# yuanzhi-zhu/DiffPIR

Hardware: AMD Instinct MI355X
Metric: restored images/sec @100 NFE, 256x256 (higher is better)
Workload: dtype f32 (GEMMs as 3 x f16 MFMA on hi/lo-split fp32 operands, fp32 accumulate; exact-fp32-MFMA mode in alt_precision); 1 GPU; configs[1]: ffhq topology 256x256 deblur (61x61 Gaussian PSF), 100 NFE, batch 16/GPU, device Philox noise, hipGraph=on; global_batch=16, nfe=100, collective=none

## Files before the change

### diffpir_amd/_lib.py

```python
from __future__ import annotations

import ctypes as C
import os

_HERE = os.path.dirname(os.path.abspath(__file__))
LIB_PATH = os.environ.get("DIFFPIR_LIB") or os.path.join(_HERE, "csrc", "libdiffpir_hip.so")
ABI_VERSION = 2



class UNetDesc(C.Structure):
    _fields_ = [("image_size", C.c_int32), ("in_channels", C.c_int32), ("model_channels", C.c_int32),
                ("out_channels", C.c_int32), ("num_res_blocks", C.c_int32), ("num_head_channels", C.c_int32),
                ("n_channel_mult", C.c_int32), ("channel_mult", C.c_float * 8),
                ("n_attention_ds", C.c_int32), ("attention_ds", C.c_int32 * 8), ("num_classes", C.c_int32)]


class Tensor(C.Structure):
    _fields_ = [("name", C.c_char_p), ("data", C.c_void_p), ("ndim", C.c_int32), ("shape", C.c_int64 * 4)]


class Step(C.Structure):
    _fields_ = [("t", C.c_int32), ("last", C.c_int32), ("c1", C.c_float), ("c2", C.c_float), ("tau", C.c_float),
                ("sa_t", C.c_float), ("s1m_t", C.c_float), ("sa_p", C.c_float),
                ("k1", C.c_float), ("q", C.c_float), ("es", C.c_float), ("k2", C.c_float)]


class LoopDesc(C.Structure):
    _fields_ = [("task", C.c_int32), ("B", C.c_int32), ("H", C.c_int32), ("W", C.c_int32), ("sf", C.c_int32),
                ("kh", C.c_int32), ("kw", C.c_int32), ("in_iter", C.c_int32), ("gamma", C.c_float),
                ("guidance", C.c_float), ("sa_start", C.c_float), ("s1m_start", C.c_float),
                ("y_dev", C.c_void_p), ("k_dev", C.c_void_p), ("mask_dev", C.c_void_p), ("labels_host", C.c_void_p),
                ("noise_init_dev", C.c_void_p), ("noise_n1_dev", C.c_void_p), ("noise_n2_dev", C.c_void_p),
                ("seed", C.c_uint64), ("image_offset", C.c_int64), ("use_graph", C.c_int32),
                ("skip_dead_final_eval", C.c_int32), ("generate_mode", C.c_int32), ("first_order", C.c_int32),
                ("noise_rp_dev", C.c_void_p), ("ddim_sample", C.c_int32)]


class InpaintRow(C.Structure):
    _fields_ = [("t", C.c_int32), ("last", C.c_int32), ("pos", C.c_int32), ("back", C.c_int32),
                ("c1", C.c_float), ("c2", C.c_float), ("tau", C.c_float), ("sa_t", C.c_float), ("s1m_t", C.c_float), ("sa_p", C.c_float),
                ("k1", C.c_float), ("q", C.c_float), ("es", C.c_float), ("k2", C.c_float),
                ("sae", C.c_float), ("sb", C.c_float), ("sa_n", C.c_float), ("s1m_n", C.c_float),
                ("mix_next", C.c_int32), ("reserved", C.c_int32)]


class DpsCoef(C.Structure):
    _fields_ = [("pc1", C.c_float), ("pc2", C.c_float), ("min_log", C.c_float), ("max_log", C.c_float), ("sa_prev", C.c_float), ("s1m_prev", C.c_float)]


class PSampleCoef(C.Structure):
    _fields_ = [("c1", C.c_float), ("c2", C.c_float), ("pc1", C.c_float), ("pc2", C.c_float), ("min_log", C.c_float), ("max_log", C.c_float),
                ("ddim", C.c_int32), ("sa_prev", C.c_float), ("s1m_prev", C.c_float)]


class DegradeDesc(C.Structure):
    _fields_ = [("task", C.c_int32), ("B", C.c_int32), ("H", C.c_int32), ("W", C.c_int32), ("sf", C.c_int32),
                ("kh", C.c_int32), ("kw", C.c_int32), ("noise_level_img", C.c_float), ("seed", C.c_uint64), ("image_offset", C.c_int64)]


class Conv3Desc(C.Structure):
    _fields_ = ([(n, C.c_int32) for n in ("B", "ca", "cb", "Cout", "H", "W", "mode", "res_mode", "scaled", "prologue", "route", "split",
                                          "defer", "Cout2")] +
                [(n, C.c_void_p) for n in ("xa", "xb", "w", "bias", "res", "prm", "gamma", "beta", "film", "gamma2", "beta2", "w2", "bias2",
                                           "out", "stat_out", "out2")] +
                [(n, C.c_int32) for n in ("stat_kind_out", "path_out", "ksplit_out", "reserved")])


class Conv9Desc(C.Structure):
    _fields_ = ([(n, C.c_int32) for n in ("B", "Cin", "Cout", "H", "W", "res_mode", "hop", "Cout2")] +
                [(n, C.c_void_p) for n in ("x", "w", "bias", "res", "prm", "gamma2", "beta2", "film2", "w2", "bias2", "out", "stat_out", "out2")] +
                [(n, C.c_int32) for n in ("ran_out", "iters")] + [("ms_out", C.c_double)])


PROF_CLASSES = 8
PROF_NAMES = ["conv3x3", "conv1x1", "groupnorm_stats", "attention", "fft_prox", "elementwise", "unet_forward", "loop_graph"]

SIGNATURES = {
    "dpir_version": (C.c_int, []),
    "dpir_device_count": (C.c_int, [C.POINTER(C.c_int)]),
    "dpir_create": (C.c_int, [C.c_int, C.POINTER(C.c_void_p)]),
    "dpir_destroy": (None, [C.c_void_p]),
    "dpir_last_error": (C.c_char_p, [C.c_void_p]),
    "dpir_sync": (C.c_int, [C.c_void_p]),
    "dpir_stream": (C.c_void_p, [C.c_void_p]),
    "dpir_malloc": (C.c_int, [C.c_void_p, C.c_size_t, C.POINTER(C.c_void_p)]),
    "dpir_free": (C.c_int, [C.c_void_p, C.c_void_p]),
    "dpir_h2d": (C.c_int, [C.c_void_p, C.c_void_p, C.c_void_p, C.c_size_t]),
    "dpir_d2h": (C.c_int, [C.c_void_p, C.c_void_p, C.c_void_p, C.c_size_t]),
    "dpir_d2d": (C.c_int, [C.c_void_p, C.c_void_p, C.c_void_p, C.c_size_t]),
    "dpir_load_unet": (C.c_int, [C.c_void_p, C.POINTER(UNetDesc), C.POINTER(Tensor), C.c_int]),
    "dpir_set_precision": (C.c_int, [C.c_void_p, C.c_int]),
    "dpir_unet_forward": (C.c_int, [C.c_void_p, C.c_void_p, C.c_void_p, C.c_void_p, C.c_void_p, C.c_int, C.c_int, C.c_int]),
    "dpir_model_fn_xstart": (C.c_int, [C.c_void_p, C.c_void_p, C.c_int, C.c_float, C.c_float, C.c_void_p, C.c_void_p,
                                       C.c_int, C.c_int, C.c_int]),
    "dpir_enable_grad": (C.c_int, [C.c_void_p, C.c_int]),
    "dpir_unet_vjp": (C.c_int, [C.c_void_p, C.c_void_p, C.c_void_p, C.c_void_p, C.c_void_p, C.c_void_p, C.c_void_p, C.c_int, C.c_int, C.c_int]),
    "dpir_run_dps_loop": (C.c_int, [C.c_void_p, C.POINTER(LoopDesc), C.POINTER(Step), C.POINTER(DpsCoef), C.c_int, C.c_int, C.c_float,
                                    C.c_void_p, C.c_void_p, C.c_float, C.c_void_p, C.c_void_p]),
    "dpir_p_sample": (C.c_int, [C.c_void_p, C.c_void_p, C.c_int, C.POINTER(PSampleCoef), C.c_void_p, C.c_void_p, C.c_void_p, C.c_void_p, C.c_int, C.c_int, C.c_int]),
    "dpir_eps_from_xstart": (C.c_int, [C.c_void_p, C.c_void_p, C.c_void_p, C.c_float, C.c_float, C.c_int, C.c_void_p, C.c_size_t]),
    "dpir_grad_and_value": (C.c_int, [C.c_void_p, C.c_int, C.c_void_p, C.c_void_p, C.c_int, C.c_void_p, C.c_void_p, C.c_int, C.c_int, C.c_int]),
    "dpir_blur_reflect": (C.c_int, [C.c_void_p, C.c_void_p, C.c_void_p, C.c_int, C.c_int, C.c_float, C.c_float, C.c_void_p, C.c_int, C.c_int, C.c_int]),
    "dpir_blur_reflect_adjoint": (C.c_int, [C.c_void_p, C.c_void_p, C.c_void_p, C.c_int, C.c_int, C.c_float, C.c_void_p, C.c_int, C.c_int, C.c_int]),
    "dpir_grad_and_value_blur": (C.c_int, [C.c_void_p, C.c_int, C.c_void_p, C.c_void_p, C.c_void_p, C.c_int, C.c_int, C.c_void_p, C.c_void_p,
                                           C.c_int, C.c_int, C.c_int]),
    "dpir_run_deblur_grad_loop": (C.c_int, [C.c_void_p, C.POINTER(LoopDesc), C.POINTER(Step), C.POINTER(DpsCoef), C.c_int, C.c_int, C.c_float,
                                            C.c_void_p, C.c_void_p, C.c_void_p, C.c_void_p]),
    "dpir_unet_read_tap": (C.c_int, [C.c_void_p, C.c_char_p, C.c_void_p, C.c_size_t, C.POINTER(C.c_size_t)]),
    "dpir_prox_fft_precalc": (C.c_int, [C.c_void_p, C.c_void_p, C.c_void_p, C.c_int, C.c_int, C.c_int, C.c_int, C.c_int,
                                        C.c_int, C.POINTER(C.c_void_p)]),
    "dpir_prox_free": (None, [C.c_void_p, C.c_void_p]),
    "dpir_prox_read": (C.c_int, [C.c_void_p, C.c_void_p, C.c_int, C.c_void_p, C.c_size_t]),
    "dpir_data_solution": (C.c_int, [C.c_void_p, C.c_void_p, C.c_void_p, C.c_float, C.c_void_p]),
    "dpir_prox_fft_apply": (C.c_int, [C.c_void_p, C.c_void_p, C.c_void_p, C.c_float, C.c_float]),
    "dpir_set_prox_launch": (C.c_int, [C.c_void_p, C.c_int]),
    "dpir_prox_fft_apply_timed": (C.c_int, [C.c_void_p, C.c_void_p, C.c_void_p, C.c_float, C.c_float, C.c_int, C.c_int, C.POINTER(C.c_float)]),
    "dpir_prox_mask": (C.c_int, [C.c_void_p, C.c_void_p, C.c_void_p, C.c_void_p, C.c_float, C.c_float, C.c_int, C.c_int, C.c_int]),
    "dpir_resize_down": (C.c_int, [C.c_void_p, C.c_void_p, C.c_void_p, C.c_int, C.c_int, C.c_int, C.c_int]),
    "dpir_prox_ibp": (C.c_int, [C.c_void_p, C.c_void_p, C.c_void_p, C.c_float, C.c_float, C.c_int, C.c_int, C.c_int, C.c_int, C.c_int]),
    "dpir_bicubic_up": (C.c_int, [C.c_void_p, C.c_void_p, C.c_void_p, C.c_int, C.c_int, C.c_int, C.c_int]),
    "dpir_renoise": (C.c_int, [C.c_void_p, C.c_void_p, C.c_void_p, C.POINTER(Step), C.c_void_p, C.c_void_p, C.c_int, C.c_int, C.c_int]),
    "dpir_repaint_mix": (C.c_int, [C.c_void_p, C.c_void_p, C.c_void_p, C.c_void_p, C.c_void_p, C.c_void_p, C.c_int, C.c_int, C.c_int]),
    "dpir_finalize": (C.c_int, [C.c_void_p, C.c_void_p, C.c_void_p, C.c_void_p, C.c_int, C.c_int, C.c_int]),
    "dpir_randn": (C.c_int, [C.c_void_p, C.c_void_p, C.c_uint64, C.c_uint64, C.c_int64, C.c_int, C.c_int, C.c_int, C.c_int]),
    "dpir_ewise": (C.c_int, [C.c_void_p, C.c_int, C.c_void_p, C.c_void_p, C.c_size_t, C.c_float, C.c_void_p, C.c_size_t]),
    "dpir_comm_unique_id": (C.c_int, [C.c_void_p]),
    "dpir_comm_version": (C.c_int, [C.POINTER(C.c_int)]),
    "dpir_device_info": (C.c_int, [C.c_void_p, C.c_char_p, C.c_size_t]),
    "dpir_comm_init": (C.c_int, [C.c_void_p, C.c_int, C.c_int, C.c_void_p]),
    "dpir_allgather_results": (C.c_int, [C.c_void_p, C.c_void_p, C.c_void_p, C.c_size_t]),
    "dpir_comm_allreduce_max": (C.c_int, [C.c_void_p, C.POINTER(C.c_double)]),
    "dpir_comm_barrier": (C.c_int, [C.c_void_p]),
    "dpir_comm_destroy": (C.c_int, [C.c_void_p]),
    "dpir_degrade": (C.c_int, [C.c_void_p, C.POINTER(DegradeDesc), C.c_void_p, C.c_void_p, C.c_void_p, C.c_void_p, C.c_void_p]),
    "dpir_metrics": (C.c_int, [C.c_void_p, C.c_void_p, C.c_void_p, C.c_int, C.c_int, C.c_int, C.c_void_p, C.c_void_p]),
    "dpir_run_loop": (C.c_int, [C.c_void_p, C.POINTER(LoopDesc), C.POINTER(Step), C.c_int, C.c_void_p, C.c_void_p]),
    "dpir_inpaint_step": (C.c_int, [C.c_void_p, C.c_void_p, C.c_void_p, C.c_int, C.c_void_p, C.c_void_p, C.POINTER(InpaintRow), C.c_int, C.c_float,
                                    C.c_void_p, C.c_void_p, C.c_void_p, C.c_void_p, C.c_uint64, C.c_int64, C.c_int, C.c_void_p, C.c_int, C.c_int, C.c_int]),
    "dpir_run_inpaint_loop": (C.c_int, [C.c_void_p, C.POINTER(LoopDesc), C.POINTER(InpaintRow), C.c_int, C.c_void_p, C.c_void_p, C.c_void_p]),
    "dpir_prof_enable": (C.c_int, [C.c_void_p, C.c_int]),
    "dpir_prof_reset": (C.c_int, [C.c_void_p]),
    "dpir_prof_read": (C.c_int, [C.c_void_p, C.POINTER(C.c_double), C.POINTER(C.c_int64)]),
    "dpir_graph_cache_size": (C.c_int, [C.c_void_p]),
    "dpir_unet_flops": (C.c_double, [C.c_void_p, C.c_int, C.c_int]),
    "dpir_unet_flops_class": (C.c_double, [C.c_void_p, C.c_int, C.c_int, C.c_int]),
}

_lib = None


class EngineLibraryError(RuntimeError):
    pass


DEBUG_LIB_PATH = os.path.join(_HERE, "csrc", "libdiffpir_dbg.so")
_dbg = None


def load_debug():
    global _dbg
    if _dbg is not None:
        return _dbg
    load()
    if not os.path.exists(DEBUG_LIB_PATH):
        raise EngineLibraryError(f"{DEBUG_LIB_PATH} not found: `make -C diffpir_amd/csrc` builds it next to the product library")
    d = C.CDLL(DEBUG_LIB_PATH)
    d.dpir_debug_conv_bench.argtypes = [C.c_void_p] + [C.c_int] * 10 + [C.POINTER(C.c_double)]
    d.dpir_debug_conv7_emit_supported.argtypes = [C.c_void_p] + [C.c_int] * 4 + [C.POINTER(C.c_int)]
    d.dpir_debug_victim.argtypes = [C.c_void_p, C.c_int, C.c_int, C.c_int, C.c_longlong, C.c_int, C.POINTER(C.c_ulonglong)]
    d.dpir_debug_victim_alu.argtypes = [C.c_void_p, C.c_int, C.c_int, C.c_int, C.c_int, C.POINTER(C.c_ulonglong)]
    for fn in (d.dpir_debug_victim_fft_pk, d.dpir_debug_victim_fft_nopk):
        fn.argtypes = [C.c_void_p, C.c_int, C.c_int, C.c_int, C.POINTER(C.c_ulonglong)]
    d.dpir_debug_conv7_check.argtypes = [C.c_void_p] + [C.c_int] * 10 + [C.POINTER(C.c_double), C.POINTER(C.c_double), C.POINTER(C.c_ulonglong),
                                                                        C.POINTER(C.c_float), C.POINTER(C.c_int)]
    d.dpir_debug_conv5_layer.argtypes = [C.c_void_p] + [C.c_int] * 7 + [C.c_void_p] * 7 + [C.POINTER(C.c_int)]
    d.dpir_debug_conv5_layer.restype = C.c_int
    d.dpir_debug_conv3_layer.argtypes = [C.c_void_p, C.POINTER(Conv3Desc)]
    d.dpir_debug_conv3_layer.restype = C.c_int
    d.dpir_debug_conv9_layer.argtypes = [C.c_void_p, C.POINTER(Conv9Desc)]
    d.dpir_debug_conv9_layer.restype = C.c_int
    for n in ("dpir_debug_conv_bench", "dpir_debug_victim", "dpir_debug_victim_alu", "dpir_debug_victim_fft_pk", "dpir_debug_victim_fft_nopk",
              "dpir_debug_conv7_check"):
        getattr(d, n).restype = C.c_int
    _dbg = d
    return d


def load():
    global _lib
    if _lib is not None:
        return _lib
    if not os.path.exists(LIB_PATH):
        raise EngineLibraryError(
            f"{LIB_PATH} not found: build it with `python -c 'import __graft_entry__ as g; g.build()'` "
            f"or `make -C diffpir_amd/csrc`.  There is no CPU fallback.")
    try:
        import torch
    except ImportError:
        pass
    try:
        lib = C.CDLL(LIB_PATH)
    except OSError as ex:
        raise EngineLibraryError(f"cannot load {LIB_PATH}: {ex}") from ex
    for name, (res, args) in SIGNATURES.items():
        try:
            fn = getattr(lib, name)
        except AttributeError as ex:
            raise EngineLibraryError(f"{LIB_PATH} does not export {name}") from ex
        fn.restype = res
        fn.argtypes = args
    if lib.dpir_version() != ABI_VERSION:
        raise EngineLibraryError("ABI version mismatch")
    _lib = lib
    return lib
```

### diffpir_amd/csrc/dbg_conv.hip

```cpp
#include "engine.h"
#include "conv6_params.h"
#include "conv9.h"
#include "../../include/diffpir_debug.h"
#include <string.h>
#include <vector>
using namespace dpir;
static int fail(dpir_engine* e, const Status& s) {
    if (e) e->last_error = s.msg;
    return s.code;
}
#define API_TRY(e, expr)                          \
    do {                                          \
        Status _s = (expr);                       \
        if (!_s.ok()) return fail((e), _s);       \
    } while (0)
#define API_HIP(e, expr)                                                                  \
    do {                                                                                  \
        hipError_t _h = (expr);                                                           \
        if (_h != hipSuccess)                                                             \
            return fail((e), Status{DPIR_ERR_HIP, std::string(#expr) + ": " + hipGetErrorString(_h)}); \
    } while (0)

__global__ void dbg_bitdiff_kernel(const float* a, const float* b, size_t n, unsigned long long* out) {
    unsigned long long cnt = 0; unsigned mx = 0;
    for (size_t i = (size_t)blockIdx.x * blockDim.x + threadIdx.x; i < n; i += (size_t)gridDim.x * blockDim.x) {
        const float x = a[i], y = b[i];
        if (__builtin_bit_cast(unsigned, x) != __builtin_bit_cast(unsigned, y)) {
            ++cnt;
            const float d = fabsf(x - y);
            const unsigned u = d == d ? __builtin_bit_cast(unsigned, d) : 0x7fc00000u;
            mx = u > mx ? u : mx;
        }
    }
    if (cnt) { atomicAdd(&out[0], cnt); atomicMax(&out[1], (unsigned long long)mx); }
}

extern "C" {
int dpir_debug_conv_bench(dpir_engine* e, int B, int Cin, int Cout, int H, int W, int ks, int mode, int with_prm,
                          int dbg, int iters, double* ms_out) {
    if (!e || !ms_out || iters <= 0) return DPIR_ERR_INVALID;
    (void)hipSetDevice(e->device);
    int taps = ks * ks, coutp = round_up(Cout, 64), cinp = round_up(Cin, 16);
    float *x = nullptr, *w = nullptr, *bias = nullptr, *out = nullptr, *partial = nullptr; float4* prm = nullptr;
    API_TRY(e, e->ws.getT("dbg#x", (size_t)B * Cin * H * W, &x));
    API_TRY(e, e->ws.getT("dbg#w", (size_t)cinp * taps * coutp, &w));
    API_TRY(e, e->ws.getT("dbg#b", (size_t)coutp, &bias));
    API_TRY(e, e->ws.getT("dbg#o", (size_t)B * Cout * H * W, &out));
    API_TRY(e, e->ws.getT("dbg#prm", (size_t)B * Cin, &prm));
    API_TRY(e, e->ws.getT("conv#partial", (size_t)16 * 1024 * 1024, &partial));
    API_TRY(e, launch_randn(e->stream, x, 1, 1, 0, 1, (size_t)B * Cin * H * W));
    API_TRY(e, launch_randn(e->stream, w, 2, 1, 0, 1, (size_t)cinp * taps * coutp));
    API_TRY(e, launch_randn(e->stream, bias, 3, 1, 0, 1, (size_t)coutp));
    API_TRY(e, launch_randn(e->stream, reinterpret_cast<float*>(prm), 4, 1, 0, 1, (size_t)B * Cin * 4));
    ConvArgs a;
    a.src.a = x; a.src.ca = Cin; a.src.Hs = H; a.src.Ws = W; a.src.mode = 0; a.src.prm = with_prm ? prm : nullptr;
    a.w = w; a.bias = bias; a.out = out; a.B = B; a.Cin = Cin; a.Cout = Cout; a.CoutP = coutp; a.H = H; a.W = W; a.ks = ks;
    a.partial = partial; a.partial_capacity = (size_t)16 * 1024 * 1024;
    const void* w16 = nullptr; float w16_scale = 1.f;
    if (dbg != 0) {
        std::vector<float> hw((size_t)Cout * Cin * taps);
        for (size_t i = 0; i < hw.size(); ++i) hw[i] = (float)((i * 2654435761u) % 2001) / 1000.0f * 0.05f - 0.05f;
        std::vector<uint16_t> w16v;
        w16_scale = ks == 1 ? pack_weights_f16x3_1x1(hw.data(), Cout, Cin, w16v) : pack_weights_conv6(hw.data(), Cout, Cin, w16v);
        void* wp = nullptr;
        API_TRY(e, e->ws.get("dbg#w16", w16v.size() * 2, &wp));
        API_HIP(e, hipMemcpy(wp, w16v.data(), w16v.size() * 2, hipMemcpyHostToDevice));
        w16 = wp;
    }
    Conv5Args a5;
    Conv6Args a6;
    const bool use5 = dbg != 0 && ks == 1, use6 = dbg != 0 && ks == 3;
    if (use5) {
        a5.src = CatSrc{x, Cin, nullptr, 0}; a5.prm = a.src.prm; a5.w16 = w16; a5.w16_scale = w16_scale; a5.bias = bias; a5.out = out;
        a5.B = B; a5.Cout = Cout; a5.H = H; a5.W = W; a5.x1 = e->precision == 2;
    }
    if (use6) {
        int C8 = 2 * ((Cin + 15) / 16);
        size_t plane = (size_t)B * C8 * H * W * 16;
        char* s16 = nullptr;
        API_TRY(e, e->ws.getT("dbg#s16", 2 * plane, &s16));
        API_TRY(e, launch_act_split(e->stream, CatSrc{x, Cin, nullptr, 0}, a.src.prm, 0, B, H, W, s16, s16 + plane));
        a6.xhi = s16; a6.xlo = s16 + plane; a6.w16 = w16; a6.w16_scale = w16_scale; a6.bias = bias; a6.out = out;
        a6.B = B; a6.Cin = Cin; a6.Cout = Cout; a6.H = H; a6.W = W; a6.partial = partial; a6.partial_capacity = a.partial_capacity;
        a6.x1 = e->precision == 2;
    }
    auto run_once = [&]() -> Status {
        if (use5) return launch_conv5(e->stream, a5);
        if (use6) {
            if (dbg == 1) DPIR_TRY(launch_act_split(e->stream, CatSrc{x, Cin, nullptr, 0}, a.src.prm, 0, B, H, W, const_cast<void*>(a6.xhi), const_cast<void*>(a6.xlo)));
            return launch_conv6(e->stream, a6);
        }
        return launch_conv(e->stream, a);
    };
    API_TRY(e, run_once());
    hipEvent_t e0, e1;
    API_HIP(e, hipEventCreate(&e0)); API_HIP(e, hipEventCreate(&e1));
    API_HIP(e, hipEventRecord(e0, e->stream));
    for (int i = 0; i < iters; ++i) API_TRY(e, run_once());
    API_HIP(e, hipEventRecord(e1, e->stream));
    API_HIP(e, hipEventSynchronize(e1));
    float ms = 0; API_HIP(e, hipEventElapsedTime(&ms, e0, e1));
    (void)hipEventDestroy(e0); (void)hipEventDestroy(e1);
    *ms_out = ms / iters;
    return DPIR_OK;
}

int dpir_debug_conv7_check(dpir_engine* e, int B, int Cin, int Cout, int H, int W, int res_mode, int x1, int split, int scaled, int iters,
                            double* ms6_out, double* ms7_out, unsigned long long* mismatches_out, float* maxdiff_out, int* ksplit_out) {
    if (!e || !ms6_out || !ms7_out || !mismatches_out || !maxdiff_out || !ksplit_out || iters <= 0 || res_mode < -1 || res_mode > 2) return DPIR_ERR_INVALID;
    (void)hipSetDevice(e->device);
    if (!conv6_supported(H, W) || W < 32) return fail(e, invalid("conv7 check: conv6 only has the 8 x 32 geometry (W >= 32) to compare with"));
    const size_t nx = (size_t)B * Cin * H * W, no = (size_t)B * Cout * H * W;
    const size_t nres = res_mode == 1 ? no / 4 : (res_mode == 2 ? no * 4 : no);
    const int slots = conv6_stat_slots(H, W);
    const size_t nst = (size_t)B * Cout * slots;
    const size_t pcap = (size_t)16 * no;
    float *x = nullptr, *bias = nullptr, *o6 = nullptr, *o7 = nullptr, *res = nullptr, *p6 = nullptr, *p7 = nullptr, *scale = nullptr;
    float2 *st6 = nullptr, *st7 = nullptr;
    unsigned long long* cmp = nullptr;
    API_TRY(e, e->ws.getT("c7#x", nx, &x));
    API_TRY(e, e->ws.getT("c7#b", (size_t)round_up(Cout, 64), &bias));
    API_TRY(e, e->ws.getT("c7#o6", no, &o6));
    API_TRY(e, e->ws.getT("c7#o7", no, &o7));
    API_TRY(e, e->ws.getT("c7#res", nres, &res));
    API_TRY(e, e->ws.getT("c7#st6", nst, &st6));
    API_TRY(e, e->ws.getT("c7#st7", nst, &st7));
    API_TRY(e, e->ws.getT("c7#cmp", (size_t)2, &cmp));
    API_TRY(e, e->ws.getT("c7#scale", (size_t)4, &scale));
    if (split) { API_TRY(e, e->ws.getT("c7#p6", pcap, &p6)); API_TRY(e, e->ws.getT("c7#p7", pcap, &p7)); }
    API_TRY(e, launch_randn(e->stream, x, 11, 1, 0, 1, nx));
    API_TRY(e, launch_randn(e->stream, bias, 12, 1, 0, 1, (size_t)round_up(Cout, 64)));
    API_TRY(e, launch_randn(e->stream, res, 13, 1, 0, 1, nres));
    const float quarter = 0.25f;
    API_HIP(e, hipMemcpyAsync(scale, &quarter, 4, hipMemcpyHostToDevice, e->stream));
    std::vector<float> hw((size_t)Cout * Cin * 9);
    for (size_t i = 0; i < hw.size(); ++i) hw[i] = (float)((i * 2654435761u) % 2001) / 1000.0f * 0.05f - 0.05f;
    std::vector<uint16_t> w16v;
    const float w16_scale = pack_weights_conv6(hw.data(), Cout, Cin, w16v);
    void* wp = nullptr;
    API_TRY(e, e->ws.get("c7#w16", w16v.size() * 2, &wp));
    API_HIP(e, hipMemcpy(wp, w16v.data(), w16v.size() * 2, hipMemcpyHostToDevice));
    const int chunks = (Cin + 15) / 16, C8 = 2 * chunks;
    const size_t plane = (size_t)B * C8 * H * W * 16;
    char* s16 = nullptr;
    API_TRY(e, e->ws.getT("c7#s16", 2 * plane, &s16));
    API_TRY(e, launch_act_split(e->stream, CatSrc{x, Cin, nullptr, 0}, nullptr, 0, B, H, W, s16, x1 ? nullptr : s16 + plane));
    Conv6Args a6;
    a6.xhi = s16; a6.xlo = x1 ? nullptr : s16 + plane; a6.w16 = wp; a6.w16_scale = w16_scale; a6.bias = bias;
    a6.B = B; a6.Cin = Cin; a6.Cout = Cout; a6.H = H; a6.W = W; a6.x1 = x1 != 0;
    if (res_mode >= 0) { a6.res = res; a6.res_mode = res_mode; }
    if (scaled) a6.out_scale_dev = scale;
    a6.out = o6; a6.stat = st6; a6.force_kernel = 6;
    if (split) { a6.partial = p6; a6.partial_capacity = pcap; }
    Conv6K k;
    k.xhi = reinterpret_cast<const char*>(a6.xhi); k.xlo = reinterpret_cast<const char*>(a6.xlo);
    k.w16 = reinterpret_cast<const char*>(wp); k.bias = bias; k.out = o7; k.res = a6.res; k.res_mode = a6.res_mode;
    k.B = B; k.Cout = Cout; k.H = H; k.W = W; k.n_chunks_total = chunks; k.C8 = C8;
    k.out_scale = 1.0f / w16_scale; k.out_scale_dev = a6.out_scale_dev; k.zeros = nullptr;
    const int geo = W >= 32 ? 0 : (W >= 16 ? 1 : 2);
    const int tw = geo == 0 ? 32 : (geo == 1 ? 16 : 8), th = geo == 0 ? 8 : (geo == 1 ? 16 : 8), ti = geo == 2 ? 4 : 1;
    k.tiles_x = (W + tw - 1) / tw; k.tiles_y = (H + th - 1) / th;
    const int n_ptiles = k.tiles_x * k.tiles_y * ((B + ti - 1) / ti);
    k.n_co_blocks = (Cout + 127) / 128;
    const int blocks = n_ptiles * k.n_co_blocks;
    int S = 1;
    if (split && blocks < 384) {
        S = (512 + blocks - 1) / blocks;
        if (S > chunks / 2) S = chunks / 2;
        if (S > 16) S = 16;
        if (S < 1) S = 1;
        if ((size_t)S * no > pcap) S = 1;
    }
    k.chunks_per_split = (chunks + S - 1) / S;
    S = (chunks + k.chunks_per_split - 1) / k.chunks_per_split;
    k.ksplit = S; k.partial = S > 1 ? p7 : nullptr;
    k.stat = S == 1 ? st7 : nullptr; k.stat_slots = S == 1 ? slots : 0;
    *ksplit_out = S;
    API_HIP(e, hipMemsetAsync(o6, 0xFF, no * 4, e->stream));
    API_HIP(e, hipMemsetAsync(o7, 0x7F, no * 4, e->stream));
    API_HIP(e, hipMemsetAsync(st6, 0xFF, nst * 8, e->stream));
    API_HIP(e, hipMemsetAsync(st7, 0x7F, nst * 8, e->stream));
    if (split) { API_HIP(e, hipMemsetAsync(p6, 0xFF, (size_t)S * no * 4, e->stream)); API_HIP(e, hipMemsetAsync(p7, 0x7F, (size_t)S * no * 4, e->stream)); }
    API_HIP(e, hipMemsetAsync(cmp, 0, 16, e->stream));
    int k6 = 0;
    PendingConv pend;
    API_TRY(e, launch_conv6(e->stream, a6, &k6, &pend));
    if ((S > 1) != (k6 == 3) || (S > 1 && pend.ksplit != S)) return fail(e, Status{DPIR_ERR_INVALID, "conv7 check: the split rule of launch_conv6 changed"});
    API_TRY(e, launch_conv7(e->stream, k, blocks * S, x1 != 0));
    API_HIP(e, hipGetLastError());
    if (S > 1) {
        hipLaunchKernelGGL(dbg_bitdiff_kernel, dim3(2048), dim3(256), 0, e->stream, p6, p7, (size_t)S * no, cmp);
    } else {
        hipLaunchKernelGGL(dbg_bitdiff_kernel, dim3(2048), dim3(256), 0, e->stream, o6, o7, no, cmp);
        hipLaunchKernelGGL(dbg_bitdiff_kernel, dim3(256), dim3(256), 0, e->stream, reinterpret_cast<const float*>(st6), reinterpret_cast<const float*>(st7), nst * 2, cmp);
    }
    unsigned long long h[2] = {0, 0};
    API_HIP(e, hipMemcpyAsync(h, cmp, 16, hipMemcpyDeviceToHost, e->stream));
    API_HIP(e, hipStreamSynchronize(e->stream));
    *mismatches_out = h[0];
    const unsigned mb = (unsigned)h[1];
    *maxdiff_out = __builtin_bit_cast(float, mb);
    hipEvent_t e0, e1, e2;
    API_HIP(e, hipEventCreate(&e0)); API_HIP(e, hipEventCreate(&e1)); API_HIP(e, hipEventCreate(&e2));
    for (int i = 0; i < 3; ++i) { API_TRY(e, launch_conv6(e->stream, a6, &k6, &pend)); API_TRY(e, launch_conv7(e->stream, k, blocks * S, x1 != 0)); }
    API_HIP(e, hipEventRecord(e0, e->stream));
    for (int i = 0; i < iters; ++i) API_TRY(e, launch_conv6(e->stream, a6, &k6, &pend));
    API_HIP(e, hipEventRecord(e1, e->stream));
    for (int i = 0; i < iters; ++i) API_TRY(e, launch_conv7(e->stream, k, blocks * S, x1 != 0));
    API_HIP(e, hipEventRecord(e2, e->stream));
    API_HIP(e, hipEventSynchronize(e2));
    float m6 = 0, m7 = 0;
    API_HIP(e, hipEventElapsedTime(&m6, e0, e1)); API_HIP(e, hipEventElapsedTime(&m7, e1, e2));
    (void)hipEventDestroy(e0); (void)hipEventDestroy(e1); (void)hipEventDestroy(e2);
    *ms6_out = m6 / iters; *ms7_out = m7 / iters;
    return DPIR_OK;
}

int dpir_debug_conv5_layer(dpir_engine* e, int B, int ca, int cb, int Cout, int H, int W, int tile, const float* xa, const float* xb,
                           const float* w, const float* bias, const float* prm, const float* res, float* out, int* path_out) {
    if (!e || !xa || !w || !bias || !out || !path_out || B <= 0 || ca <= 0 || cb < 0 || (cb > 0 && !xb) || Cout <= 0 || tile < 0 || tile > 2) return DPIR_ERR_INVALID;
    if (e->precision == 0) return fail(e, invalid("conv5 layer: the engine is in f32 mode"));
    (void)hipSetDevice(e->device);
    const int C = ca + cb, HW = H * W;
    const size_t na = (size_t)B * ca * HW, nb = (size_t)B * cb * HW, no = (size_t)B * Cout * HW;
    float *dxa = nullptr, *dxb = nullptr, *dbias = nullptr, *dout = nullptr, *dres = nullptr, *dw = nullptr, *partial = nullptr; float4* dprm = nullptr;
    API_TRY(e, e->ws.getT("c5#xa", na, &dxa));
    API_TRY(e, e->ws.getT("c5#xb", nb + 1, &dxb));
    API_TRY(e, e->ws.getT("c5#b", (size_t)round_up(Cout, 64), &dbias));
    API_TRY(e, e->ws.getT("c5#o", no, &dout));
    API_TRY(e, e->ws.getT("c5#res", no, &dres));
    API_TRY(e, e->ws.getT("c5#prm", (size_t)B * C, &dprm));
    API_HIP(e, hipMemcpy(dxa, xa, na * 4, hipMemcpyHostToDevice));
    if (cb) API_HIP(e, hipMemcpy(dxb, xb, nb * 4, hipMemcpyHostToDevice));
    API_HIP(e, hipMemset(dbias, 0, (size_t)round_up(Cout, 64) * 4));
    API_HIP(e, hipMemcpy(dbias, bias, (size_t)Cout * 4, hipMemcpyHostToDevice));
    if (prm) API_HIP(e, hipMemcpy(dprm, prm, (size_t)B * C * 16, hipMemcpyHostToDevice));
    if (res) API_HIP(e, hipMemcpy(dres, res, no * 4, hipMemcpyHostToDevice));
    API_HIP(e, hipMemset(dout, 0xFF, no * 4));
    std::vector<uint16_t> w16v;
    const float w16_scale = pack_weights_f16x3_1x1(w, Cout, C, w16v);
    void* wp = nullptr;
    API_TRY(e, e->ws.get("c5#w16", w16v.size() * 2, &wp));
    API_HIP(e, hipMemcpy(wp, w16v.data(), w16v.size() * 2, hipMemcpyHostToDevice));
    const bool has_prm = prm != nullptr;
    const bool use5 = !(has_prm && C % 16) && (tile != 0 || conv5_supported(B, Cout, H, W, has_prm) || conv5_small_supported(B, ca, cb, Cout, H, W, has_prm));
    Status st;
    if (use5) {
        Conv5Args a5;
        a5.src = CatSrc{dxa, ca, cb ? dxb : nullptr, cb}; a5.prm = has_prm ? dprm : nullptr; a5.w16 = wp; a5.w16_scale = w16_scale;
        a5.bias = dbias; a5.out = dout; a5.res = res ? dres : nullptr; a5.B = B; a5.Cout = Cout; a5.H = H; a5.W = W;
        a5.x1 = e->precision == 2; a5.force_tile = tile;
        *path_out = tile ? tile : (conv5_small_supported(B, ca, cb, Cout, H, W, has_prm) ? 2 : 1);
        st = launch_conv5(e->stream, a5);
    } else {
        const int coutp = round_up(Cout, 64), cinp = round_up(C, 16);
        std::vector<float> packed((size_t)cinp * coutp, 0.f);
        for (int co = 0; co < Cout; ++co)
            for (int ci = 0; ci < C; ++ci) packed[(size_t)ci * coutp + co] = w[(size_t)co * C + ci];
        API_TRY(e, e->ws.getT("c5#w", packed.size(), &dw));
        API_HIP(e, hipMemcpy(dw, packed.data(), packed.size() * 4, hipMemcpyHostToDevice));
        API_TRY(e, e->ws.getT("conv#partial", (size_t)16 * 1024 * 1024, &partial));
        ConvArgs a;
        a.src.a = dxa; a.src.ca = ca; a.src.b = cb ? dxb : nullptr; a.src.cb = cb; a.src.Hs = H; a.src.Ws = W; a.src.mode = 0;
        a.src.prm = has_prm ? dprm : nullptr;
        a.w = dw; a.bias = dbias; a.out = dout; a.res = res ? dres : nullptr; a.res_mode = 0;
        a.B = B; a.Cin = C; a.Cout = Cout; a.CoutP = coutp; a.H = H; a.W = W; a.ks = 1;
        a.partial = partial; a.partial_capacity = (size_t)16 * 1024 * 1024;
        *path_out = 0;
        st = launch_conv(e->stream, a);
    }
    API_TRY(e, st);
    API_HIP(e, hipStreamSynchronize(e->stream));
    API_HIP(e, hipMemcpy(out, dout, no * 4, hipMemcpyDeviceToHost));
    return DPIR_OK;
}

int dpir_debug_conv3_layer(dpir_engine* e, dpir_debug_conv3_desc* d) {
    if (!e || !d) return DPIR_ERR_INVALID;
    d->path_out = -1; d->ksplit_out = 0; d->stat_kind_out = 0;
    const int B = d->B, ca = d->ca, cb = d->cb, Cout = d->Cout, H = d->H, W = d->W, mode = d->mode, C = ca + cb;
    if (!d->xa || !d->w || !d->bias || !d->out || B <= 0 || ca <= 0 || cb < 0 || (cb > 0 && !d->xb) || Cout <= 0 || H <= 0 || W <= 0 || mode < 0 || mode > 2 ||
        d->res_mode < -1 || d->res_mode > 2 || (d->res_mode >= 0 && !d->res) || d->prologue < 0 || d->prologue > 2 ||
        (d->route != 0 && d->route != 6 && d->route != 7 && d->route != 8))
        return fail(e, invalid("conv3 layer: bad descriptor"));
    if (d->prologue == 1 && !d->prm) return fail(e, invalid("conv3 layer: prologue 1 needs the table"));
    if (d->prologue == 2 && (!d->gamma || !d->beta)) return fail(e, invalid("conv3 layer: prologue 2 needs gamma and beta"));
    if (mode == 1 && ((H | W) & 1)) return fail(e, invalid("conv3 layer: a nearest-up source needs an even output size"));
    if (d->res_mode == 1 && ((H | W) & 1)) return fail(e, invalid("conv3 layer: a half-resolution residual needs an even output size"));
    if (d->defer && (!d->split || (d->route != 0 && d->route != 7) || !d->gamma2 || !d->beta2 || !d->w2 || !d->bias2 || !d->out2 || d->Cout2 <= 0))
        return fail(e, invalid("conv3 layer: defer needs split, route 0 or 7 and the second stage's operands"));
    (void)hipSetDevice(e->device);
    const int Hs = mode == 1 ? H / 2 : (mode == 2 ? H * 2 : H), Ws = mode == 1 ? W / 2 : (mode == 2 ? W * 2 : W);
    const size_t HWs = (size_t)Hs * Ws, HW = (size_t)H * W;
    const size_t na = (size_t)B * ca * HWs, nb = (size_t)B * cb * HWs, no = (size_t)B * Cout * HW;
    const size_t nres = d->res_mode == 1 ? no / 4 : (d->res_mode == 2 ? no * 4 : no);
    const int coutp = round_up(Cout, 64);
    float *dxa = nullptr, *dxb = nullptr, *dbias = nullptr, *dout = nullptr, *dres = nullptr, *scale = nullptr; float4* dprm = nullptr;
    API_TRY(e, e->ws.getT("c3#xa", na, &dxa));
    API_TRY(e, e->ws.getT("c3#xb", nb + 1, &dxb));
    API_TRY(e, e->ws.getT("c3#b", (size_t)coutp, &dbias));
    API_TRY(e, e->ws.getT("c3#o", no, &dout));
    API_TRY(e, e->ws.getT("c3#res", nres, &dres));
    API_TRY(e, e->ws.getT("c3#prm", (size_t)B * C, &dprm));
    API_TRY(e, e->ws.getT("c3#scale", (size_t)4, &scale));
    API_HIP(e, hipMemcpy(dxa, d->xa, na * 4, hipMemcpyHostToDevice));
    if (cb) API_HIP(e, hipMemcpy(dxb, d->xb, nb * 4, hipMemcpyHostToDevice));
    API_HIP(e, hipMemset(dbias, 0, (size_t)coutp * 4));
    API_HIP(e, hipMemcpy(dbias, d->bias, (size_t)Cout * 4, hipMemcpyHostToDevice));
    if (d->prologue == 1) API_HIP(e, hipMemcpy(dprm, d->prm, (size_t)B * C * 16, hipMemcpyHostToDevice));
    if (d->res_mode >= 0) API_HIP(e, hipMemcpy(dres, d->res, nres * 4, hipMemcpyHostToDevice));
    const float quarter = 0.25f;
    API_HIP(e, hipMemcpy(scale, &quarter, 4, hipMemcpyHostToDevice));
    API_HIP(e, hipMemset(dout, 0xFF, no * 4));
    const float* res = d->res_mode >= 0 ? dres : nullptr;
    const int res_mode = d->res_mode >= 0 ? d->res_mode : 0;
    const CatSrc src{dxa, ca, cb ? dxb : nullptr, cb};
    const bool x1 = e->precision == 2;
    const bool f16path = e->precision != 0 && conv6_supported(H, W);
    const size_t pcap = (size_t)16 * no;
    float* partial = nullptr;
    if (d->split) {
        API_TRY(e, e->ws.getT("c3#partial", pcap, &partial));
        API_HIP(e, hipMemset(partial, 0xFF, pcap * 4));
    }

    if (d->route == 8) {
        if (e->precision == 0) return fail(e, invalid("conv3 layer: conv8 needs an f16 engine"));
        if (d->prologue != 1 || cb || mode != 0 || res || d->scaled || d->split) return fail(e, invalid("conv3 layer: conv8 takes a table prologue, one source, no resampling, no residual"));
        if (!conv8_supported(B, C, Cout, H, W)) return fail(e, invalid("conv8: shape not supported"));
        std::vector<uint16_t> w8;
        const float w8_scale = pack_weights_conv8(d->w, Cout, C, w8);
        void* wp = nullptr;
        API_TRY(e, e->ws.get("c3#w8", w8.size() * 2, &wp));
        API_HIP(e, hipMemcpy(wp, w8.data(), w8.size() * 2, hipMemcpyHostToDevice));
        Conv8Args a8;
        a8.x = dxa; a8.prm = dprm; a8.w = wp; a8.w_scale = w8_scale; a8.bias = dbias; a8.out = dout;
        a8.B = B; a8.C = C; a8.Cout = Cout; a8.H = H; a8.W = W; a8.range_ctr = e->range_ctr; a8.x1 = x1;
        a8.silu = d->prm[3] != 0.f;
        API_TRY(e, launch_conv8(e->stream, a8));
        API_HIP(e, hipStreamSynchronize(e->stream));
        API_HIP(e, hipMemcpy(d->out, dout, no * 4, hipMemcpyDeviceToHost));
        d->path_out = 8;
        return DPIR_OK;
    }

    if (!f16path) {
        if (d->route != 0) return fail(e, invalid("conv3 layer: conv6 / conv7 cannot be forced here (f32 engine or a shape the f16 path refuses)"));
        if (d->prologue == 2) return fail(e, Status{DPIR_ERR_UNSUPPORTED, "conv3 layer: gn_act_small only feeds the f16 path"});
        if (d->scaled || d->defer) return fail(e, invalid("conv3 layer: the fp32 kernel has no device output scale and no deferred combine"));
        const int cinp = round_up(C, 16);
        std::vector<float> packed((size_t)cinp * 9 * coutp, 0.f);
        for (int co = 0; co < Cout; ++co)
            for (int ci = 0; ci < C; ++ci)
                for (int t = 0; t < 9; ++t) packed[((size_t)ci * 9 + t) * coutp + co] = d->w[((size_t)co * C + ci) * 9 + t];
        float* dw = nullptr;
        API_TRY(e, e->ws.getT("c3#w", packed.size(), &dw));
        API_HIP(e, hipMemcpy(dw, packed.data(), packed.size() * 4, hipMemcpyHostToDevice));
        ConvArgs a;
        a.src.a = dxa; a.src.ca = ca; a.src.b = cb ? dxb : nullptr; a.src.cb = cb; a.src.Hs = Hs; a.src.Ws = Ws; a.src.mode = mode;
        a.src.prm = d->prologue == 1 ? dprm : nullptr;
        a.w = dw; a.bias = dbias; a.out = dout; a.res = res; a.res_mode = res_mode;
        a.B = B; a.Cin = C; a.Cout = Cout; a.CoutP = coutp; a.H = H; a.W = W; a.ks = 3;
        a.partial = partial; a.partial_capacity = partial ? pcap : 0;
        API_TRY(e, launch_conv(e->stream, a));
        API_HIP(e, hipStreamSynchronize(e->stream));
        API_HIP(e, hipMemcpy(d->out, dout, no * 4, hipMemcpyDeviceToHost));
        d->path_out = 0;
        return DPIR_OK;
    }

    const int C8 = 2 * ((C + 15) / 16);
    const size_t plane = (size_t)B * C8 * HW * 16;
    char* s16 = nullptr;
    API_TRY(e, e->ws.getT("c3#s16", 2 * plane, &s16));
    API_HIP(e, hipMemset(s16, 0xFF, 2 * plane));
    if (d->prologue == 2) {
        if (C % 16 || !gn_act_small_supported(C, Hs, Ws, mode)) return fail(e, Status{DPIR_ERR_UNSUPPORTED, "conv3 layer: gn_act_small refuses this shape"});
        float *dg = nullptr, *db = nullptr, *df = nullptr;
        API_TRY(e, e->ws.getT("c3#gamma", (size_t)C, &dg));
        API_TRY(e, e->ws.getT("c3#beta", (size_t)C, &db));
        API_TRY(e, e->ws.getT("c3#film", (size_t)B * 2 * C, &df));
        API_HIP(e, hipMemcpy(dg, d->gamma, (size_t)C * 4, hipMemcpyHostToDevice));
        API_HIP(e, hipMemcpy(db, d->beta, (size_t)C * 4, hipMemcpyHostToDevice));
        if (d->film) API_HIP(e, hipMemcpy(df, d->film, (size_t)B * 2 * C * 4, hipMemcpyHostToDevice));
        GnActArgs ga;
        ga.src = src; ga.gamma = dg; ga.beta = db;
        ga.film = d->film ? df : nullptr; ga.film_stride = 2 * C; ga.film_off = 0; ga.fstep = nullptr; ga.frows = 2 * C;
        ga.silu = true; ga.mode = mode; ga.B = B; ga.Hs = Hs; ga.Ws = Ws;
        ga.hi = s16; ga.lo = x1 ? nullptr : s16 + plane; ga.range_ctr = e->range_ctr;
        API_TRY(e, launch_gn_act_small(e->stream, ga));
    } else {
        API_TRY(e, launch_act_split(e->stream, src, d->prologue == 1 ? dprm : nullptr, mode, B, H, W, s16, x1 ? nullptr : s16 + plane, e->range_ctr));
    }
    std::vector<uint16_t> w16v;
    const float w16_scale = pack_weights_conv6(d->w, Cout, C, w16v);
    void* wp = nullptr;
    API_TRY(e, e->ws.get("c3#w16", w16v.size() * 2, &wp));
    API_HIP(e, hipMemcpy(wp, w16v.data(), w16v.size() * 2, hipMemcpyHostToDevice));
    Conv6Args a6;
    a6.x1 = x1;
    a6.xhi = s16; a6.xlo = s16 + plane; a6.w16 = wp; a6.w16_scale = w16_scale;
    a6.bias = dbias; a6.out = dout; a6.res = res; a6.res_mode = res_mode;
    a6.B = B; a6.Cin = C; a6.Cout = Cout; a6.H = H; a6.W = W;
    a6.partial = partial; a6.partial_capacity = partial ? pcap : 0;
    a6.force_kernel = d->route;
    if (d->scaled) a6.out_scale_dev = scale;
    const int slots = conv6_stat_slots(H, W);
    float2* st = nullptr; double2* sp = nullptr;
    const size_t nst = (size_t)B * Cout * slots;
    if (slots > 0 && Cout % 32 == 0) {
        API_TRY(e, e->ws.getT("c3#st", nst, &st));
        API_TRY(e, e->ws.getT("c3#sp", (size_t)B * Cout, &sp));
        API_HIP(e, hipMemset(st, 0xFF, nst * 8));
        API_HIP(e, hipMemset(sp, 0xFF, (size_t)B * Cout * 16));
    }
    a6.stat = st; a6.stat_plane = sp;
    int kind = 0, kernel = 0;
    PendingConv pc;
    API_TRY(e, launch_conv6(e->stream, a6, &kind, d->defer ? &pc : nullptr, &kernel));
    d->path_out = kernel; d->stat_kind_out = kind;
    d->ksplit_out = kind == 3 ? pc.ksplit : 1;
    if (d->split && !d->defer) {
        PendingConv probe;
        Conv6Args b6 = a6;
        float* o2 = nullptr;
        API_TRY(e, e->ws.getT("c3#o_again", no, &o2));
        b6.out = o2;
        int k2 = 0;
        API_HIP(e, hipStreamSynchronize(e->stream));
        std::vector<float> first(no);
        API_HIP(e, hipMemcpy(first.data(), dout, no * 4, hipMemcpyDeviceToHost));
        API_TRY(e, launch_conv6(e->stream, b6, &k2, &probe));
        d->ksplit_out = k2 == 3 ? probe.ksplit : 1;
        if (k2 == 3) API_TRY(e, launch_conv6_resolve(e->stream, probe));
        API_HIP(e, hipStreamSynchronize(e->stream));
        std::vector<float> again(no);
        API_HIP(e, hipMemcpy(again.data(), o2, no * 4, hipMemcpyDeviceToHost));
        if (memcmp(first.data(), again.data(), no * 4) != 0) return fail(e, Status{DPIR_ERR_STATE, "conv3 layer: two identical split-K launches disagree"});
    }
    if (d->defer) {
        if (kind != 3) return fail(e, invalid("conv3 layer: defer was asked for but launch_conv6 did not split this launch"));
        const int Cn = Cout, Co2 = d->Cout2;
        if (Cn % 16 || !gn_act_small_supported(Cn, H, W, 0)) return fail(e, Status{DPIR_ERR_UNSUPPORTED, "conv3 layer: gn_act_small refuses the second stage"});
        const int C8b = 2 * ((Cn + 15) / 16);
        const size_t plane2 = (size_t)B * C8b * HW * 16, no2 = (size_t)B * Co2 * HW;
        char* s16b = nullptr; float *dg = nullptr, *db = nullptr, *dbias2 = nullptr, *dout2 = nullptr;
        API_TRY(e, e->ws.getT("c3#s16b", 2 * plane2, &s16b));
        API_TRY(e, e->ws.getT("c3#gamma2", (size_t)Cn, &dg));
        API_TRY(e, e->ws.getT("c3#beta2", (size_t)Cn, &db));
        API_TRY(e, e->ws.getT("c3#b2", (size_t)round_up(Co2, 64), &dbias2));
        API_TRY(e, e->ws.getT("c3#o2", no2, &dout2));
        API_HIP(e, hipMemset(s16b, 0xFF, 2 * plane2));
        API_HIP(e, hipMemcpy(dg, d->gamma2, (size_t)Cn * 4, hipMemcpyHostToDevice));
        API_HIP(e, hipMemcpy(db, d->beta2, (size_t)Cn * 4, hipMemcpyHostToDevice));
        API_HIP(e, hipMemset(dbias2, 0, (size_t)round_up(Co2, 64) * 4));
        API_HIP(e, hipMemcpy(dbias2, d->bias2, (size_t)Co2 * 4, hipMemcpyHostToDevice));
        API_HIP(e, hipMemset(dout2, 0xFF, no2 * 4));
        GnActArgs ga;
        ga.src = CatSrc{dout, Cn, nullptr, 0}; ga.pend = pc; ga.gamma = dg; ga.beta = db;
        ga.silu = true; ga.mode = 0; ga.B = B; ga.Hs = H; ga.Ws = W;
        ga.hi = s16b; ga.lo = x1 ? nullptr : s16b + plane2; ga.range_ctr = e->range_ctr;
        API_TRY(e, launch_gn_act_small(e->stream, ga));
        std::vector<uint16_t> w16b;
        const float w16b_scale = pack_weights_conv6(d->w2, Co2, Cn, w16b);
        void* wp2 = nullptr;
        API_TRY(e, e->ws.get("c3#w16b", w16b.size() * 2, &wp2));
        API_HIP(e, hipMemcpy(wp2, w16b.data(), w16b.size() * 2, hipMemcpyHostToDevice));
        Conv6Args c6;
        c6.x1 = x1; c6.xhi = s16b; c6.xlo = s16b + plane2; c6.w16 = wp2; c6.w16_scale = w16b_scale;
        c6.bias = dbias2; c6.out = dout2; c6.B = B; c6.Cin = Cn; c6.Cout = Co2; c6.H = H; c6.W = W;
        API_TRY(e, launch_conv6(e->stream, c6));
        API_HIP(e, hipStreamSynchronize(e->stream));
        API_HIP(e, hipMemcpy(d->out2, dout2, no2 * 4, hipMemcpyDeviceToHost));
    }
    API_HIP(e, hipStreamSynchronize(e->stream));
    API_HIP(e, hipMemcpy(d->out, dout, no * 4, hipMemcpyDeviceToHost));
    if (d->stat_out && (kind == 1 || kind == 2)) {
        if (kind == 1) {
            std::vector<float2> hs(nst);
            API_HIP(e, hipMemcpy(hs.data(), st, nst * 8, hipMemcpyDeviceToHost));
            for (size_t pl = 0; pl < (size_t)B * Cout; ++pl) {
                double s1 = 0.0, s2 = 0.0;
                for (int k = 0; k < slots; ++k) { s1 += (double)hs[pl * slots + k].x; s2 += (double)hs[pl * slots + k].y; }
                d->stat_out[2 * pl] = s1; d->stat_out[2 * pl + 1] = s2;
            }
        } else {
            API_HIP(e, hipMemcpy(d->stat_out, sp, (size_t)B * Cout * 16, hipMemcpyDeviceToHost));
        }
    }
    return DPIR_OK;
}

int dpir_debug_conv9_layer(dpir_engine* e, dpir_debug_conv9_desc* d) {
    if (!e || !d) return DPIR_ERR_INVALID;
    d->ran_out = 0;
    const int B = d->B, Cin = d->Cin, Cout = d->Cout, H = d->H, W = d->W;
    if (!d->x || !d->w || !d->bias || B <= 0 || Cin <= 0 || Cout <= 0 || H <= 0 || W <= 0 || d->res_mode < -1 || d->res_mode > 2 ||
        (d->res_mode >= 0 && !d->res) || (!d->hop && !d->out) || (d->hop && (!d->gamma2 || !d->beta2 || !d->w2 || !d->bias2 || !d->out2 || d->Cout2 <= 0)))
        return fail(e, invalid("conv9 layer: bad descriptor"));
    if (e->grad_enabled) return fail(e, Status{DPIR_ERR_UNSUPPORTED, "conv9 layer: a gradient-mode engine keeps launch_conv6's route"});
    if (e->precision == 0) return fail(e, Status{DPIR_ERR_UNSUPPORTED, "conv9 layer: the f32 precision keeps the fp32 kernel"});
    if (d->hop && d->res_mode >= 0) return fail(e, invalid("conv9 layer: the hop's first layer takes no residual"));
    if ((d->res_mode == 1 && ((H | W) & 1))) return fail(e, invalid("conv9 layer: a half-resolution residual needs an even output size"));
    (void)hipSetDevice(e->device);
    const bool x1 = e->precision == 2;
    const size_t HW = (size_t)H * W, nx = (size_t)B * Cin * HW, no = (size_t)B * Cout * HW;
    const size_t nres = d->res_mode == 1 ? no / 4 : (d->res_mode == 2 ? no * 4 : no);
    const int chunks = (Cin + 15) / 16, C8 = 2 * chunks;
    const size_t plane = (size_t)B * C8 * HW * 16;
    float *dx = nullptr, *dbias = nullptr, *dout = nullptr, *dres = nullptr; float4* dprm = nullptr; double2* sp = nullptr; char* s16 = nullptr;
    API_TRY(e, e->ws.getT("c9#x", nx, &dx));
    API_TRY(e, e->ws.getT("c9#b", (size_t)round_up(Cout, 64), &dbias));
    API_TRY(e, e->ws.getT("c9#o", no, &dout));
    API_TRY(e, e->ws.getT("c9#res", nres, &dres));
    API_TRY(e, e->ws.getT("c9#prm", (size_t)B * Cin, &dprm));
    API_TRY(e, e->ws.getT("c9#sp", (size_t)B * Cout, &sp));
    API_TRY(e, e->ws.getT("c9#s16", 2 * plane, &s16));
    API_HIP(e, hipMemcpy(dx, d->x, nx * 4, hipMemcpyHostToDevice));
    API_HIP(e, hipMemset(dbias, 0, (size_t)round_up(Cout, 64) * 4));
    API_HIP(e, hipMemcpy(dbias, d->bias, (size_t)Cout * 4, hipMemcpyHostToDevice));
    if (d->prm) API_HIP(e, hipMemcpy(dprm, d->prm, (size_t)B * Cin * 16, hipMemcpyHostToDevice));
    if (d->res_mode >= 0) API_HIP(e, hipMemcpy(dres, d->res, nres * 4, hipMemcpyHostToDevice));
    API_HIP(e, hipMemsetAsync(dout, 0xFF, no * 4, e->stream));
    API_HIP(e, hipMemsetAsync(sp, 0xFF, (size_t)B * Cout * 16, e->stream));
    API_HIP(e, hipMemsetAsync(s16, 0xFF, 2 * plane, e->stream));
    API_TRY(e, launch_act_split(e->stream, CatSrc{dx, Cin, nullptr, 0}, d->prm ? dprm : nullptr, 0, B, H, W, s16, x1 ? nullptr : s16 + plane, e->range_ctr));
    std::vector<uint16_t> w16v;
    const float w16_scale = pack_weights_conv6(d->w, Cout, Cin, w16v);
    void* wp = nullptr;
    API_TRY(e, e->ws.get("c9#w16", w16v.size() * 2, &wp));
    API_HIP(e, hipMemcpy(wp, w16v.data(), w16v.size() * 2, hipMemcpyHostToDevice));
    Conv9Args a9;
    a9.xhi = s16; a9.xlo = s16 + plane; a9.w16 = wp; a9.w16_scale = w16_scale; a9.bias = dbias; a9.out = dout;
    if (d->res_mode >= 0) { a9.res = dres; a9.res_mode = d->res_mode; }
    a9.B = B; a9.Cin = Cin; a9.Cout = Cout; a9.H = H; a9.W = W; a9.stat_plane = sp; a9.x1 = x1;
    d->ms_out = 0.0;
    auto timed = [&](auto&& launch) -> int {
        if (d->iters <= 0) return DPIR_OK;
        hipEvent_t e0, e1;
        API_HIP(e, hipEventCreate(&e0)); API_HIP(e, hipEventCreate(&e1));
        API_HIP(e, hipEventRecord(e0, e->stream));
        for (int i = 0; i < d->iters; ++i) API_TRY(e, launch());
        API_HIP(e, hipEventRecord(e1, e->stream));
        API_HIP(e, hipEventSynchronize(e1));
        float ms = 0; API_HIP(e, hipEventElapsedTime(&ms, e0, e1));
        (void)hipEventDestroy(e0); (void)hipEventDestroy(e1);
        d->ms_out = ms / d->iters;
        return DPIR_OK;
    };
    if (!d->hop) {
        API_TRY(e, launch_conv9(e->stream, a9));
        if (int rc = timed([&]() { return launch_conv9(e->stream, a9); })) return rc;
        API_HIP(e, hipStreamSynchronize(e->stream));
        d->ran_out = 1;
        API_HIP(e, hipMemcpy(d->out, dout, no * 4, hipMemcpyDeviceToHost));
        if (d->stat_out) API_HIP(e, hipMemcpy(d->stat_out, sp, (size_t)B * Cout * 16, hipMemcpyDeviceToHost));
        return DPIR_OK;
    }
    const int Co2 = d->Cout2, C8b = 2 * ((Cout + 15) / 16);
    const size_t plane2 = (size_t)B * C8b * HW * 16, no2 = (size_t)B * Co2 * HW;
    char* s16b = nullptr; float *dg = nullptr, *db = nullptr, *df = nullptr, *dbias2 = nullptr, *dout2 = nullptr;
    API_TRY(e, e->ws.getT("c9#s16b", 2 * plane2, &s16b));
    API_TRY(e, e->ws.getT("c9#gamma2", (size_t)Cout, &dg));
    API_TRY(e, e->ws.getT("c9#beta2", (size_t)Cout, &db));
    API_TRY(e, e->ws.getT("c9#film2", (size_t)B * 2 * Cout, &df));
    API_TRY(e, e->ws.getT("c9#b2", (size_t)round_up(Co2, 64), &dbias2));
    API_TRY(e, e->ws.getT("c9#o2", no2, &dout2));
    API_HIP(e, hipMemsetAsync(s16b, 0xFF, 2 * plane2, e->stream));
    API_HIP(e, hipMemcpy(dg, d->gamma2, (size_t)Cout * 4, hipMemcpyHostToDevice));
    API_HIP(e, hipMemcpy(db, d->beta2, (size_t)Cout * 4, hipMemcpyHostToDevice));
    if (d->film2) API_HIP(e, hipMemcpy(df, d->film2, (size_t)B * 2 * Cout * 4, hipMemcpyHostToDevice));
    API_HIP(e, hipMemset(dbias2, 0, (size_t)round_up(Co2, 64) * 4));
    API_HIP(e, hipMemcpy(dbias2, d->bias2, (size_t)Co2 * 4, hipMemcpyHostToDevice));
    API_HIP(e, hipMemsetAsync(dout2, 0xFF, no2 * 4, e->stream));
    std::vector<uint16_t> w16b;
    const float w16b_scale = pack_weights_conv6(d->w2, Co2, Cout, w16b);
    void* wp2 = nullptr;
    API_TRY(e, e->ws.get("c9#w16b", w16b.size() * 2, &wp2));
    API_HIP(e, hipMemcpy(wp2, w16b.data(), w16b.size() * 2, hipMemcpyHostToDevice));
    Conv6Emit em;
    em.hi = s16b; em.lo = x1 ? nullptr : s16b + plane2; em.C8 = C8b; em.gamma = dg; em.beta = db;
    em.film = d->film2 ? df : nullptr; em.film_stride = 2 * Cout; em.film_off = 0; em.frows = 2 * Cout; em.fstep = nullptr;
    em.range_ctr = e->range_ctr;
    a9.out = nullptr; a9.stat_plane = nullptr; a9.emit = &em;
    API_TRY(e, launch_conv9(e->stream, a9));
    Conv9Args b9;
    b9.xhi = s16b; b9.xlo = s16b + plane2; b9.w16 = wp2; b9.w16_scale = w16b_scale; b9.bias = dbias2; b9.out = dout2;
    b9.B = B; b9.Cin = Cout; b9.Cout = Co2; b9.H = H; b9.W = W; b9.x1 = x1;
    API_TRY(e, launch_conv9(e->stream, b9));
    if (int rc = timed([&]() -> Status { DPIR_TRY(launch_conv9(e->stream, a9)); return launch_conv9(e->stream, b9); })) return rc;
    API_HIP(e, hipStreamSynchronize(e->stream));
    d->ran_out = 1;
    API_HIP(e, hipMemcpy(d->out2, dout2, no2 * 4, hipMemcpyDeviceToHost));
    return DPIR_OK;
}

int dpir_debug_conv7_emit_supported(dpir_engine* e, int B, int Cout, int H, int W, int* capacity_out) {
    if (!e) return 0;
    (void)hipSetDevice(e->device);
    if (capacity_out) *capacity_out = conv7_emit_capacity();
    return conv7_emit_supported(B, Cout, H, W) ? 1 : 0;
}

}
```

### diffpir_amd/csrc/engine.h

```cpp
#pragma once
#include <functional>
#include "common.h"
#include "elem.h"
#include "prox.h"

namespace dpir {

struct DevBuf {
    void* p = nullptr;
    size_t bytes = 0;
};

struct Workspace {
    std::map<std::string, DevBuf> bufs;
    size_t total = 0;
    bool frozen = false;
    uint64_t generation = 0;
    Status get(const std::string& name, size_t bytes, void** out);
    template <class T> Status getT(const std::string& name, size_t count, T** out) {
        void* p = nullptr;
        DPIR_TRY(get(name, count * sizeof(T), &p));
        *out = reinterpret_cast<T*>(p);
        return Status{};
    }
    void release();
};

struct ConvW { float* w = nullptr; float* bias = nullptr; int cin = 0, cout = 0, coutp = 0, ks = 3;
               void* w16 = nullptr; float w16_scale = 1.f;
               float* wT = nullptr; int coutpT = 0;
               void* w8 = nullptr; float w8_scale = 1.f;
               void* w16T = nullptr; float w16T_scale = 1.f; };
struct GnW { float* gamma = nullptr; float* beta = nullptr; int c = 0; };
struct ResW {
    std::string name;
    int cin = 0, cout = 0, mode = 0;
    GnW gn1; ConvW conv1; GnW gn2; ConvW conv2;
    bool has_skip = false; ConvW skip;
    int film_off = 0;
};
struct AttnW { std::string name; int c = 0; GnW norm; ConvW qkv; ConvW proj; };
struct Layer { int kind; int idx; std::string name; };
typedef std::vector<Layer> Block;

struct UNet {
    bool loaded = false;
    dpir_unet_desc desc{};
    std::vector<float> cm;
    std::vector<Block> in_blocks, out_blocks;
    Block mid;
    ConvW conv_in;
    std::vector<ResW> res;
    std::vector<AttnW> attn;
    GnW out_gn; ConvW out_conv;
    float *te_w0 = nullptr, *te_b0 = nullptr, *te_w2 = nullptr, *te_b2 = nullptr, *label_emb = nullptr, *freqs = nullptr;
    float *film_w = nullptr, *film_b = nullptr;
    int film_rows = 0;
    std::vector<void*> allocs;
};

struct TapInfo { const float* p; size_t numel; };

struct TapeRes { int idx; CatSrc in; int inH, inW, Ho, Wo; float* h1; float* sk; float* out; float4* prm1; float2* st1; float4* prm2; float2* st2; };
struct TapeAttn { int idx; const float* in; int H, W; float* qkv; float* att; float* out; float4* prm; float2* st; };
struct TapeNode { int kind; int idx; };
struct Tape {
    bool valid = false;
    unsigned long long serial = 0;
    int B = 0, H = 0, W = 0;
    float* conv_in_out = nullptr;
    std::vector<TapeNode> nodes; std::vector<TapeRes> res; std::vector<TapeAttn> attn;
    const float* final_h = nullptr; float4* final_prm = nullptr; float2* final_st = nullptr;
    void clear() { valid = false; nodes.clear(); res.clear(); attn.clear(); }
};

struct ResizerTab { int in_len = 0, out_len = 0, taps = 0; float* w = nullptr; int* idx = nullptr; };

}

struct dpir_prox { dpir::ProxState st; };

struct dpir_engine {
    int device = 0;
    hipStream_t stream = nullptr;
    std::string last_error;
    dpir::Profiler prof;
    dpir::UNet net;
    dpir::Workspace ws;
    std::map<std::string, dpir::TapInfo> taps;
    dpir::ProxCache prox_cache;
    std::map<std::pair<int, int>, dpir::ResizerTab> resizers;
    std::vector<void*> user_allocs;
    bool collect_taps = true;
    int precision = 0;
    bool grad_enabled = false;
    dpir::Tape tape;
    float ps_c1 = 0.f, ps_c2 = 0.f; int ps_B = 0, ps_H = 0, ps_W = 0; const float* ps_x0 = nullptr;
    unsigned long long fwd_serial = 0, ps_serial = 0;
    struct GraphKey {
        int32_t task, B, H, W, sf, in_iter, generate_mode, kind;
        int32_t host_n1, host_n2, host_rp, has_labels;
        float gamma, guidance;
        int32_t loop, loop_pad;
        uint64_t ws_generation;
    };
    struct GraphEntry { GraphKey key; hipGraphExec_t exec = nullptr; uint64_t last_use = 0; };
    std::vector<GraphEntry> graphs;
    uint64_t graph_clock = 0;
    static constexpr size_t kMaxGraphs = 16;
    dpir::ProxState loop_prox;
    void invalidate_graphs() {
        for (auto& g : graphs) if (g.exec) (void)hipGraphExecDestroy(g.exec);
        graphs.clear();
    }
    unsigned long long* range_ctr = nullptr;
    int prox_mode = 1; int cus = 256;
    bool fuse_h1_off = false;
    int fwd_since_sync = 0;
    std::function<int()> replay_last;
    unsigned long long replay_serial = 0;
    unsigned long long enqueue_serial() const { return prof.serial + copy_serial; }
    unsigned long long copy_serial = 0;
    void arm_replay(std::function<int()> fn) { ++fwd_since_sync; replay_last = std::move(fn); replay_serial = enqueue_serial(); }
    void* comm = nullptr; int comm_world = 1, comm_rank = 0;

    dpir::Status resizer(int in_len, int sf, dpir::ResizerTab* out);
};

namespace dpir {
Status unet_load(dpir_engine* e, const dpir_unet_desc* desc, const dpir_tensor* weights, int n);
void unet_free(dpir_engine* e);
Status unet_forward(dpir_engine* e, const float* x, const int* t_dev, const int* y_dev, float* out, int B, int H, int W,
                    const float* film_table = nullptr, const StepDev* film_step = nullptr, bool uniform_t = false);
Status unet_film_table(dpir_engine* e, const int* t_dev, int n_steps, float* table);
Status unet_backward(dpir_engine* e, const float* gout, float* dx);
double unet_flops(const UNet& net, int H, int W, int cls = -1);
Status comm_allreduce_sum_f64(dpir_engine* e, double* dev, size_t n);
}
```

### diffpir_amd/csrc/unet.hip

```cpp
#include "engine.h"
#include "conv6_params.h"
#include "conv9.h"
#include <unordered_map>
#include <cstdint>
#include <math.h>
#include <string.h>
#include <stdlib.h>

namespace dpir {

Status Workspace::get(const std::string& name, size_t bytes, void** out) {
    auto it = bufs.find(name);
    if (it != bufs.end() && it->second.bytes >= bytes) { *out = it->second.p; return Status{}; }
    if (frozen) return Status{DPIR_ERR_STATE, "workspace allocation of '" + name + "' during graph capture"};
    if (it != bufs.end()) { (void)hipFree(it->second.p); total -= it->second.bytes; bufs.erase(it); }
    void* p = nullptr;
    size_t rb = (bytes + 255) & ~(size_t)255;
    hipError_t err = hipMalloc(&p, rb);
    if (err != hipSuccess) return Status{DPIR_ERR_NOMEM, "hipMalloc(" + std::to_string(rb) + ") for '" + name + "' failed"};
    bufs[name] = DevBuf{p, rb};
    total += rb;
    ++generation;
    *out = p;
    return Status{};
}
void Workspace::release() {
    for (auto& kv : bufs) (void)hipFree(kv.second.p);
    bufs.clear();
    total = 0;
}

namespace {
struct WeightMap {
    std::map<std::string, const dpir_tensor*> m;
    Status find(const std::string& key, std::vector<int64_t> shape, const float** out) const {
        auto it = m.find(key);
        if (it == m.end()) return invalid("state-dict key missing: " + key);
        const dpir_tensor* t = it->second;
        if (t->ndim != (int)shape.size()) return invalid("state-dict key " + key + ": wrong rank");
        for (size_t i = 0; i < shape.size(); ++i)
            if (t->shape[i] != shape[i]) return invalid("state-dict key " + key + ": wrong shape");
        if (!t->data) return invalid("state-dict key " + key + ": null data");
        *out = t->data;
        return Status{};
    }
};

Status upload(dpir_engine* e, const float* host, size_t n, float** dev) {
    void* p = nullptr;
    if (hipMalloc(&p, n * sizeof(float)) != hipSuccess) return Status{DPIR_ERR_NOMEM, "hipMalloc for weights failed"};
    e->net.allocs.push_back(p);
    DPIR_HIP(hipMemcpy(p, host, n * sizeof(float), hipMemcpyHostToDevice));
    *dev = reinterpret_cast<float*>(p);
    return Status{};
}

Status load_conv(dpir_engine* e, const WeightMap& wm, const std::string& p, int cin, int cout, int ks, bool one_d, ConvW* out) {
    const float *w = nullptr, *b = nullptr;
    std::vector<int64_t> shape = one_d ? std::vector<int64_t>{cout, cin, 1} : std::vector<int64_t>{cout, cin, ks, ks};
    DPIR_TRY(wm.find(p + ".weight", shape, &w));
    DPIR_TRY(wm.find(p + ".bias", {cout}, &b));
    int taps = ks * ks;
    int coutp = round_up(cout, 64);
    int cinp = round_up(cin, 16);
    std::vector<float> packed((size_t)cinp * taps * coutp, 0.f);
    for (int co = 0; co < cout; ++co)
        for (int ci = 0; ci < cin; ++ci)
            for (int t = 0; t < taps; ++t)
                packed[((size_t)ci * taps + t) * coutp + co] = w[((size_t)co * cin + ci) * taps + t];
    out->cin = cin; out->cout = cout; out->coutp = coutp; out->ks = ks;
    DPIR_TRY(upload(e, packed.data(), packed.size(), &out->w));
    DPIR_TRY(upload(e, b, cout, &out->bias));
    if (e->grad_enabled) {
        const int cinT = round_up(cout, 16), coutT = round_up(cin, 64);
        std::vector<float> pt((size_t)cinT * taps * coutT, 0.f);
        for (int co = 0; co < cout; ++co)
            for (int ci = 0; ci < cin; ++ci)
                for (int t = 0; t < taps; ++t)
                    pt[((size_t)co * taps + t) * coutT + ci] = w[((size_t)co * cin + ci) * taps + (taps - 1 - t)];
        out->coutpT = coutT;
        DPIR_TRY(upload(e, pt.data(), pt.size(), &out->wT));
        if (e->precision >= 1 && (ks == 3 || ks == 1)) {
            std::vector<float> wt((size_t)cin * cout * taps);
            for (int co = 0; co < cout; ++co)
                for (int ci = 0; ci < cin; ++ci)
                    for (int t = 0; t < taps; ++t)
                        wt[((size_t)ci * cout + co) * taps + t] = w[((size_t)co * cin + ci) * taps + (taps - 1 - t)];
            std::vector<uint16_t> w16t;
            out->w16T_scale = ks == 3 ? pack_weights_conv6(wt.data(), cin, cout, w16t) : pack_weights_f16x3_1x1(wt.data(), cin, cout, w16t);
            void* pp = nullptr;
            if (hipMalloc(&pp, w16t.size() * 2) != hipSuccess) return Status{DPIR_ERR_NOMEM, "hipMalloc for the split dgrad weights failed"};
            e->net.allocs.push_back(pp);
            DPIR_HIP(hipMemcpy(pp, w16t.data(), w16t.size() * 2, hipMemcpyHostToDevice));
            out->w16T = pp;
        }
    }
    if (e->precision >= 1 && (ks == 3 || ks == 1)) {
        std::vector<uint16_t> w16;
        out->w16_scale = ks == 3 ? pack_weights_conv6(w, cout, cin, w16) : pack_weights_f16x3_1x1(w, cout, cin, w16);
        void* p = nullptr;
        if (hipMalloc(&p, w16.size() * 2) != hipSuccess) return Status{DPIR_ERR_NOMEM, "hipMalloc for split weights failed"};
        e->net.allocs.push_back(p);
        DPIR_HIP(hipMemcpy(p, w16.data(), w16.size() * 2, hipMemcpyHostToDevice));
        out->w16 = p;
        if (ks == 3 && !one_d && cout <= 16 && cin % 32 == 0) {
            std::vector<uint16_t> w8;
            out->w8_scale = pack_weights_conv8(w, cout, cin, w8);
            void* p8 = nullptr;
            if (hipMalloc(&p8, w8.size() * 2) != hipSuccess) return Status{DPIR_ERR_NOMEM, "hipMalloc for the conv8 weights failed"};
            e->net.allocs.push_back(p8);
            DPIR_HIP(hipMemcpy(p8, w8.data(), w8.size() * 2, hipMemcpyHostToDevice));
            out->w8 = p8;
        }
    }
    return Status{};
}
Status load_gn(dpir_engine* e, const WeightMap& wm, const std::string& p, int c, GnW* out) {
    const float *g = nullptr, *b = nullptr;
    if (c % 32) return invalid("GroupNorm32 channels not divisible by 32 at " + p);
    DPIR_TRY(wm.find(p + ".weight", {c}, &g));
    DPIR_TRY(wm.find(p + ".bias", {c}, &b));
    out->c = c;
    DPIR_TRY(upload(e, g, c, &out->gamma));
    DPIR_TRY(upload(e, b, c, &out->beta));
    return Status{};
}
}

void unet_free(dpir_engine* e) {
    for (void* p : e->net.allocs) (void)hipFree(p);
    e->net = UNet{};
}

Status unet_load(dpir_engine* e, const dpir_unet_desc* d, const dpir_tensor* weights, int n) {
    unet_free(e);
    UNet& net = e->net;
    net.desc = *d;
    if (d->in_channels != 3) return invalid("in_channels must be 3");
    if (d->model_channels <= 0 || d->model_channels % 32) return invalid("model_channels must be a positive multiple of 32");
    if (d->num_head_channels != 64) return Status{DPIR_ERR_UNSUPPORTED, "only num_head_channels=64 is supported"};
    if (d->n_channel_mult > 8 || d->n_attention_ds > 8) return invalid("too many channel_mult / attention_ds entries");
    if (d->n_channel_mult > 0) net.cm.assign(d->channel_mult, d->channel_mult + d->n_channel_mult);
    else if (d->image_size == 512) net.cm = {0.5f, 1, 1, 2, 2, 4, 4};
    else if (d->image_size == 256) net.cm = {1, 1, 2, 2, 4, 4};
    else if (d->image_size == 128) net.cm = {1, 1, 2, 3, 4};
    else if (d->image_size == 64) net.cm = {1, 2, 3, 4};
    else return invalid("unsupported image_size for default channel_mult");
    WeightMap wm;
    for (int i = 0; i < n; ++i) wm.m[weights[i].name] = &weights[i];

    const int mc = d->model_channels, ted = 4 * mc;
    auto has_attn = [&](int ds) { for (int i = 0; i < d->n_attention_ds; ++i) if (d->attention_ds[i] == ds) return true; return false; };
    int film_rows = 0;
    std::vector<std::pair<std::string, int>> film_parts;

    auto add_res = [&](const std::string& p, int cin, int cout, int mode, Block& blk) -> Status {
        ResW r; r.name = p; r.cin = cin; r.cout = cout; r.mode = mode;
        DPIR_TRY(load_gn(e, wm, p + ".in_layers.0", cin, &r.gn1));
        DPIR_TRY(load_conv(e, wm, p + ".in_layers.2", cin, cout, 3, false, &r.conv1));
        DPIR_TRY(load_gn(e, wm, p + ".out_layers.0", cout, &r.gn2));
        DPIR_TRY(load_conv(e, wm, p + ".out_layers.3", cout, cout, 3, false, &r.conv2));
        r.has_skip = cin != cout;
        if (r.has_skip) {
            if (mode != 0) return invalid("resampling ResBlock with channel change is not part of this architecture");
            DPIR_TRY(load_conv(e, wm, p + ".skip_connection", cin, cout, 1, false, &r.skip));
        }
        r.film_off = film_rows;
        film_rows += 2 * cout;
        film_parts.push_back({p + ".emb_layers.1", cout});
        blk.push_back(Layer{1, (int)net.res.size(), p});
        net.res.push_back(r);
        return Status{};
    };
    auto add_attn = [&](const std::string& p, int c, Block& blk) -> Status {
        AttnW a; a.name = p; a.c = c;
        if (c % 64) return invalid("attention channels not divisible by 64");
        DPIR_TRY(load_gn(e, wm, p + ".norm", c, &a.norm));
        DPIR_TRY(load_conv(e, wm, p + ".qkv", c, 3 * c, 1, true, &a.qkv));
        DPIR_TRY(load_conv(e, wm, p + ".proj_out", c, c, 1, true, &a.proj));
        blk.push_back(Layer{2, (int)net.attn.size(), p});
        net.attn.push_back(a);
        return Status{};
    };

    int ch = (int)(net.cm[0] * mc);
    const int input_ch = ch;
    {
        Block b0;
        DPIR_TRY(load_conv(e, wm, "input_blocks.0.0", 3, ch, 3, false, &net.conv_in));
        b0.push_back(Layer{0, 0, "input_blocks.0.0"});
        net.in_blocks.push_back(b0);
    }
    std::vector<int> chans{ch};
    int ds = 1;
    const int nlev = (int)net.cm.size();
    for (int level = 0; level < nlev; ++level) {
        for (int k = 0; k < d->num_res_blocks; ++k) {
            Block blk;
            std::string p = "input_blocks." + std::to_string(net.in_blocks.size());
            int cout = (int)(net.cm[level] * mc);
            DPIR_TRY(add_res(p + ".0", ch, cout, 0, blk));
            ch = cout;
            if (has_attn(ds)) DPIR_TRY(add_attn(p + ".1", ch, blk));
            net.in_blocks.push_back(blk);
            chans.push_back(ch);
        }
        if (level != nlev - 1) {
            Block blk;
            std::string p = "input_blocks." + std::to_string(net.in_blocks.size());
            DPIR_TRY(add_res(p + ".0", ch, ch, 2, blk));
            net.in_blocks.push_back(blk);
            chans.push_back(ch);
            ds *= 2;
        }
    }
    DPIR_TRY(add_res("middle_block.0", ch, ch, 0, net.mid));
    DPIR_TRY(add_attn("middle_block.1", ch, net.mid));
    DPIR_TRY(add_res("middle_block.2", ch, ch, 0, net.mid));
    for (int level = nlev - 1; level >= 0; --level) {
        for (int i = 0; i <= d->num_res_blocks; ++i) {
            Block blk;
            std::string p = "output_blocks." + std::to_string(net.out_blocks.size());
            int ich = chans.back(); chans.pop_back();
            int cout = (int)(mc * net.cm[level]);
            int j = 0;
            DPIR_TRY(add_res(p + "." + std::to_string(j++), ch + ich, cout, 0, blk));
            ch = cout;
            if (has_attn(ds)) DPIR_TRY(add_attn(p + "." + std::to_string(j++), ch, blk));
            if (level && i == d->num_res_blocks) {
                DPIR_TRY(add_res(p + "." + std::to_string(j++), ch, ch, 1, blk));
                ds /= 2;
            }
            net.out_blocks.push_back(blk);
        }
    }
    DPIR_TRY(load_gn(e, wm, "out.0", ch, &net.out_gn));
    DPIR_TRY(load_conv(e, wm, "out.2", input_ch, d->out_channels, 3, false, &net.out_conv));
    if (ch != input_ch) return invalid("final channel count mismatch");

    const float* p0 = nullptr;
    DPIR_TRY(wm.find("time_embed.0.weight", {ted, mc}, &p0)); DPIR_TRY(upload(e, p0, (size_t)ted * mc, &net.te_w0));
    DPIR_TRY(wm.find("time_embed.0.bias", {ted}, &p0)); DPIR_TRY(upload(e, p0, ted, &net.te_b0));
    DPIR_TRY(wm.find("time_embed.2.weight", {ted, ted}, &p0)); DPIR_TRY(upload(e, p0, (size_t)ted * ted, &net.te_w2));
    DPIR_TRY(wm.find("time_embed.2.bias", {ted}, &p0)); DPIR_TRY(upload(e, p0, ted, &net.te_b2));
    if (d->num_classes > 0) {
        DPIR_TRY(wm.find("label_emb.weight", {d->num_classes, ted}, &p0));
        DPIR_TRY(upload(e, p0, (size_t)d->num_classes * ted, &net.label_emb));
    }
    {
        std::vector<float> fw((size_t)film_rows * ted), fb(film_rows);
        size_t row = 0;
        for (auto& fp : film_parts) {
            const float *w = nullptr, *b = nullptr;
            DPIR_TRY(wm.find(fp.first + ".weight", {2 * fp.second, ted}, &w));
            DPIR_TRY(wm.find(fp.first + ".bias", {2 * fp.second}, &b));
            memcpy(&fw[row * ted], w, (size_t)2 * fp.second * ted * sizeof(float));
            memcpy(&fb[row], b, (size_t)2 * fp.second * sizeof(float));
            row += 2 * fp.second;
        }
        DPIR_TRY(upload(e, fw.data(), fw.size(), &net.film_w));
        DPIR_TRY(upload(e, fb.data(), fb.size(), &net.film_b));
        net.film_rows = film_rows;
    }
    {
        int half = mc / 2;
        std::vector<float> fr(half);
        for (int i = 0; i < half; ++i) {
            float arg = -(float)log(10000.0) * (float)i / (float)half;
            fr[i] = (float)exp((double)arg);
        }
        DPIR_TRY(upload(e, fr.data(), half, &net.freqs));
    }
    net.loaded = true;
    return Status{};
}

namespace {
struct Act {
    const float* a = nullptr; int ca = 0;
    const float* b = nullptr; int cb = 0;
    int H = 0, W = 0;
    int C() const { return ca + cb; }
};

struct Fwd {
    dpir_engine* e;
    hipStream_t s;
    Workspace& ws;
    int B;
    const float* film;
    int film_rows;
    int film_stride;
    const StepDev* fstep;
    float* partial;
    size_t partial_cap;
    struct FusedStat { const float2* slots; int nslots; const double2* part; };
    std::unordered_map<const float*, FusedStat> fused;
    PendingConv pending;
    bool grad = false;
    bool fuse_small;
    int emit_skip;

    Status resolve() {
        if (!pending.partial) return Status{};
        ProfScope ps(&e->prof, PC_CONV3);
        DPIR_TRY(launch_conv6_resolve(s, pending));
        if (pending.stat_plane) fused[pending.out] = FusedStat{nullptr, 0, pending.stat_plane};
        else fused.erase(pending.out);
        pending = PendingConv{};
        return Status{};
    }
    bool is_pending(const float* p) const { return pending.partial && p && p == pending.out; }

    Status gn_conv(const GnW& g, const std::string& tag, int film_off, const ConvW& cw, const Act& in, int mode,
                   const float* res, int res_mode, float* out, int Ho, int Wo, float4** prm_out = nullptr, float2** stats_out = nullptr,
                   const Conv6Emit* emit = nullptr) {
        const int C = in.C();
        const bool f16path = cw.w16 && cw.ks == 3 && conv6_supported(Ho, Wo);
        if (fuse_small && f16path && C == g.c && C % 16 == 0 && gn_act_small_supported(C, in.H, in.W, mode)) {
            const bool x1 = e->precision == 2;
            int eh = mode == 1 ? Ho / 2 : (mode == 2 ? Ho * 2 : Ho), ew = mode == 1 ? Wo / 2 : (mode == 2 ? Wo * 2 : Wo);
            if (eh != in.H || ew != in.W) return invalid("conv: source resolution does not match mode");
            if (pending.partial && !is_pending(in.a)) DPIR_TRY(resolve());
            if (is_pending(res)) return invalid("gn_conv: residual is an unfinished convolution");
            const int C8 = 2 * ((C + 15) / 16);
            const size_t plane = (size_t)B * C8 * Ho * Wo * 16;
            char* s16 = nullptr;
            DPIR_TRY(ws.getT("act#s16", 2 * plane, &s16));
            GnActArgs ga;
            ga.src = CatSrc{in.a, in.ca, in.b, in.cb};
            ga.pend = pending;
            ga.gamma = g.gamma; ga.beta = g.beta;
            ga.film = film_off >= 0 ? film : nullptr; ga.film_stride = film_stride; ga.film_off = film_off < 0 ? 0 : film_off;
            ga.fstep = fstep; ga.frows = film_rows;
            ga.silu = true; ga.mode = mode; ga.B = B; ga.Hs = in.H; ga.Ws = in.W;
            ga.hi = s16; ga.lo = x1 ? nullptr : s16 + plane; ga.range_ctr = e->range_ctr;
            if (grad) {
                DPIR_TRY(ws.getT(tag + "#prm", (size_t)B * C, &ga.prm_out));
                DPIR_TRY(ws.getT(tag + "#gst", (size_t)B * 32, &ga.stats_out));
                if (prm_out) *prm_out = ga.prm_out;
                if (stats_out) *stats_out = ga.stats_out;
            }
            {
                ProfScope ps(&e->prof, PC_ELEM);
                DPIR_TRY(launch_gn_act_small(s, ga));
            }
            if (pending.partial) { fused.erase(pending.out); pending = PendingConv{}; }
            return conv6_on_planes(cw, s16, plane, res, res_mode, out, Ho, Wo, emit);
        }
        DPIR_TRY(resolve());
        float4* prm = nullptr;
        DPIR_TRY(gn(g, in, tag, film_off, true, &prm, stats_out));
        if (prm_out) *prm_out = prm;
        return conv(cw, in, mode, prm, res, res_mode, out, Ho, Wo, emit);
    }

    bool conv9_route(const ConvW& cw, int Ho, int Wo, bool hop) const {
        static const bool on = !(getenv("DPIR_CONV9") && atoi(getenv("DPIR_CONV9")) == 0);
        static const int min_wg = getenv("DPIR_CONV9_MIN_WG") ? atoi(getenv("DPIR_CONV9_MIN_WG")) : kConv9MinWg;
        return on && !grad && e->precision != 0 && cw.w16 && cw.ks == 3 && conv9_supported(B, cw.cin, cw.cout, Ho, Wo, hop) &&
               (long long)B * (cw.cout / 32) >= min_wg;
    }

    Status conv6_on_planes(const ConvW& cw, char* s16, size_t plane, const float* res, int res_mode, float* out, int Ho, int Wo,
                           const Conv6Emit* emit = nullptr) {
        const bool x1 = e->precision == 2;
        Conv6Args a6;
        a6.x1 = x1;
        a6.xhi = s16; a6.xlo = s16 + plane; a6.w16 = cw.w16; a6.w16_scale = cw.w16_scale;
        a6.bias = cw.bias; a6.out = out; a6.res = res; a6.res_mode = res_mode;
        a6.B = B; a6.Cin = cw.cin; a6.Cout = cw.cout; a6.H = Ho; a6.W = Wo;
        a6.partial = partial; a6.partial_capacity = partial_cap;
        const int slots = conv6_stat_slots(Ho, Wo);
        float2* st = nullptr; double2* sp = nullptr;
        if (slots > 0 && cw.cout % 32 == 0) {
            const std::string key = std::to_string(reinterpret_cast<uintptr_t>(out));
            DPIR_TRY(ws.getT("st#" + key, (size_t)B * cw.cout * slots, &st));
            DPIR_TRY(ws.getT("sp#" + key, (size_t)B * cw.cout, &sp));
        }
        a6.stat = st; a6.stat_plane = sp;
        a6.emit = emit;
        if (emit) { a6.stat = nullptr; a6.stat_plane = nullptr; a6.partial = nullptr; a6.partial_capacity = 0; }
        int kind = 0;
        PendingConv pc;
        ProfScope ps(&e->prof, PC_CONV3);
        if (conv9_route(cw, Ho, Wo, emit != nullptr)) {
            Conv9Args a9;
            a9.xhi = s16; a9.xlo = s16 + plane; a9.w16 = cw.w16; a9.w16_scale = cw.w16_scale; a9.bias = cw.bias; a9.out = out;
            a9.res = res; a9.res_mode = res_mode; a9.B = B; a9.Cin = cw.cin; a9.Cout = cw.cout; a9.H = Ho; a9.W = Wo;
            a9.stat_plane = emit ? nullptr : sp; a9.x1 = x1; a9.emit = emit;
            DPIR_TRY(launch_conv9(s, a9));
            if (sp && !emit) fused[out] = FusedStat{nullptr, 0, sp};
            else fused.erase(out);
            return Status{};
        }
        DPIR_TRY(launch_conv6(s, a6, &kind, fuse_small ? &pc : nullptr));
        if (kind == 1) fused[out] = FusedStat{st, slots, nullptr};
        else if (kind == 2) fused[out] = FusedStat{nullptr, 0, sp};
        else fused.erase(out);
        if (kind == 3) pending = pc;
        return Status{};
    }

    Status conv(const ConvW& cw, const Act& in, int mode, const float4* prm, const float* res, int res_mode, float* out, int Ho, int Wo,
                const Conv6Emit* emit = nullptr) {
        const bool x1 = e->precision == 2;
        const bool use5 = cw.w16 && cw.ks == 1 && mode == 0 && (!res || res_mode == 0) && !(prm && in.C() % 16) &&
                          (conv5_supported(B, cw.cout, Ho, Wo, prm != nullptr) ||
                           conv5_small_supported(B, in.ca, in.b ? in.cb : 0, cw.cout, Ho, Wo, prm != nullptr));
        if (pending.partial && (is_pending(in.a) || is_pending(in.b) || is_pending(res) || !use5)) DPIR_TRY(resolve());
        static const bool use_conv8 = !(getenv("DPIR_CONV8") && atoi(getenv("DPIR_CONV8")) == 0);
        if (use_conv8 && cw.w8 && prm && !grad && !emit && !res && mode == 0 && !in.b && in.H == Ho && in.W == Wo &&
            conv8_supported(B, in.C(), cw.cout, Ho, Wo)) {
            Conv8Args a8;
            a8.x = in.a; a8.prm = prm; a8.w = cw.w8; a8.w_scale = cw.w8_scale; a8.bias = cw.bias; a8.out = out;
            a8.B = B; a8.C = in.C(); a8.Cout = cw.cout; a8.H = Ho; a8.W = Wo; a8.range_ctr = e->range_ctr; a8.x1 = x1;
            fused.erase(out);
            ProfScope ps(&e->prof, PC_CONV3);
            return launch_conv8(s, a8);
        }
        if (cw.w16 && cw.ks == 3 && conv6_supported(Ho, Wo)) {
            int eh = mode == 1 ? Ho / 2 : (mode == 2 ? Ho * 2 : Ho), ew = mode == 1 ? Wo / 2 : (mode == 2 ? Wo * 2 : Wo);
            if (eh != in.H || ew != in.W) return invalid("conv: source resolution does not match mode");
            const int C = in.C(), C8 = 2 * ((C + 15) / 16);
            const size_t plane = (size_t)B * C8 * Ho * Wo * 16;
            if (plane >= ((size_t)1 << 32)) return invalid("conv: split activation plane exceeds the 4 GiB buffer-descriptor range; reduce the batch");
            char* s16 = nullptr;
            DPIR_TRY(ws.getT("act#s16", 2 * plane, &s16));
            {
                ProfScope ps(&e->prof, PC_ELEM);
                DPIR_TRY(launch_act_split(s, CatSrc{in.a, in.ca, in.b, in.cb}, prm, mode, B, Ho, Wo, s16, x1 ? nullptr : s16 + plane, e->range_ctr));
            }
            return conv6_on_planes(cw, s16, plane, res, res_mode, out, Ho, Wo, emit);
        }
        if (emit) return invalid("conv: fused emission was requested for a launch that is not on the f16 3x3 path");
        if (use5) {
            Conv5Args a5;
            a5.src = CatSrc{in.a, in.ca, in.b, in.cb}; a5.prm = prm; a5.w16 = cw.w16; a5.w16_scale = cw.w16_scale;
            a5.bias = cw.bias; a5.out = out; a5.res = res; a5.B = B; a5.Cout = cw.cout; a5.H = Ho; a5.W = Wo;
            a5.range_ctr = e->range_ctr; a5.x1 = x1;
            fused.erase(out);
            ProfScope ps(&e->prof, PC_CONV1);
            return launch_conv5(s, a5);
        }
        fused.erase(out);
        ConvArgs a;
        a.src.a = in.a; a.src.ca = in.ca; a.src.b = in.b; a.src.cb = in.cb; a.src.Hs = in.H; a.src.Ws = in.W;
        a.src.mode = mode; a.src.prm = prm;
        a.w = cw.w; a.bias = cw.bias; a.out = out; a.res = res; a.res_mode = res_mode;
        a.B = B; a.Cin = cw.cin; a.Cout = cw.cout; a.CoutP = cw.coutp; a.H = Ho; a.W = Wo; a.ks = cw.ks;
        a.partial = partial; a.partial_capacity = partial_cap;
        ProfScope ps(&e->prof, cw.ks == 3 ? PC_CONV3 : PC_CONV1);
        return launch_conv(s, a);
    }
    Status gn(const GnW& g, const Act& in, const std::string& tag, int film_off, bool silu, float4** prm_out, float2** stats_out = nullptr) {
        float4* prm = nullptr;
        float2* gst = nullptr;
        if (grad) DPIR_TRY(ws.getT(tag + "#gst", (size_t)B * 32, &gst));
        if (is_pending(in.a) || is_pending(in.b)) DPIR_TRY(resolve());
        DPIR_TRY(ws.getT(tag + "#prm", (size_t)B * g.c, &prm));
        GnStatSrc src[2];
        const float* tp[2] = {in.a, in.b};
        const int tc[2] = {in.ca, in.cb};
        for (int k = 0; k < 2; ++k) {
            src[k].c = tc[k];
            if (!tp[k] || tc[k] == 0) { src[k].c = 0; continue; }
            auto it = fused.find(tp[k]);
            if (it != fused.end()) { src[k].slots = it->second.slots; src[k].nslots = it->second.nslots; src[k].part = it->second.part; continue; }
            double2* part = nullptr;
            DPIR_TRY(ws.getT(tag + "#stats" + std::to_string(k), (size_t)B * tc[k], &part));
            ProfScope ps(&e->prof, PC_GN);
            DPIR_TRY(launch_gn_stats(s, CatSrc{tp[k], tc[k], nullptr, 0}, B, in.H * in.W, part));
            src[k].part = part;
        }
        ProfScope ps(&e->prof, PC_ELEM);
        DPIR_TRY(launch_gn_prm(s, src[0], src[1], in.H * in.W, g.gamma, g.beta, film_off >= 0 ? film : nullptr, film_stride, film_off < 0 ? 0 : film_off, B, g.c, silu, prm, fstep, film_rows, gst));
        *prm_out = prm;
        if (stats_out) *stats_out = gst;
        return Status{};
    }
    void tap(const std::string& name, const float* p, size_t numel) {
        if (e->collect_taps) e->taps[name] = TapInfo{p, numel};
    }

    bool fuse_h1 = true;
    long long* fuse_arena = nullptr; size_t fuse_cap = 0, fuse_off = 0;
    bool h1_fusable(const ResW& r, int Ho, int Wo) const {
        return fuse_h1 && !grad && e->precision != 0 && r.conv1.w16 && r.conv2.w16 && r.conv1.ks == 3 && r.conv2.ks == 3 && r.gn2.c == r.cout &&
               conv7_emit_supported(B, r.cout, Ho, Wo) && fuse_arena && fuse_off + (size_t)B * 64 + (size_t)B * (r.cout / 128) <= fuse_cap &&
               (size_t)B * (2 * ((r.cout + 15) / 16)) * Ho * Wo * 16 < ((size_t)1 << 32);
    }
    Status make_emit(const ResW& r, int Ho, int Wo, Conv6Emit* em, char** s16b, size_t* plane2) {
        const bool x1 = e->precision == 2;
        const int C8 = 2 * ((r.cout + 15) / 16);
        *plane2 = (size_t)B * C8 * Ho * Wo * 16;
        DPIR_TRY(ws.getT("act#s16b", 2 * *plane2, s16b));
        em->hi = *s16b; em->lo = x1 ? nullptr : *s16b + *plane2; em->C8 = C8;
        em->gamma = r.gn2.gamma; em->beta = r.gn2.beta;
        em->film = r.film_off >= 0 ? film : nullptr; em->film_stride = film_stride; em->film_off = r.film_off < 0 ? 0 : r.film_off;
        em->frows = film_rows; em->fstep = fstep;
        em->acc = fuse_arena + fuse_off;
        fuse_off += (size_t)B * 64;
        em->cnt = reinterpret_cast<unsigned*>(fuse_arena + fuse_off);
        fuse_off += ((size_t)B * (r.cout / 128) + 1) / 2;
        em->range_ctr = e->range_ctr;
        static const int spin_env = getenv("DPIR_FUSE_SPIN_LIMIT") ? atoi(getenv("DPIR_FUSE_SPIN_LIMIT")) : 0;
        static const int extra_env = getenv("DPIR_FUSE_EXPECT_EXTRA") ? atoi(getenv("DPIR_FUSE_EXPECT_EXTRA")) : 0;
        static const int sleep_env = getenv("DPIR_FUSE_SLEEP") ? atoi(getenv("DPIR_FUSE_SLEEP")) : 5;
        em->sleep_sel = sleep_env;
        if (spin_env > 0) em->spin_limit = spin_env;
        em->expect_extra = extra_env;
        return Status{};
    }

    Status resblock(const ResW& r, const Act& in, Act* out) {
        if (in.C() != r.cin) return invalid("resblock " + r.name + ": input channels mismatch");
        int Ho = r.mode == 1 ? in.H * 2 : (r.mode == 2 ? in.H / 2 : in.H);
        int Wo = r.mode == 1 ? in.W * 2 : (r.mode == 2 ? in.W / 2 : in.W);
        if (r.mode == 2 && ((in.H | in.W) & 1)) return invalid("resblock " + r.name + ": odd size cannot be average-pooled");
        size_t on = (size_t)B * r.cout * Ho * Wo;
        float* h1 = nullptr;
        DPIR_TRY(ws.getT(r.name + "#h1", on, &h1));
        Act h1a; h1a.a = h1; h1a.ca = r.cout; h1a.H = Ho; h1a.W = Wo;
        const float* res = nullptr; int res_mode = 0;
        const int Cin = in.C();
        const size_t eplane = (size_t)B * (2 * ((Cin + 15) / 16)) * Ho * Wo * 16;
        if ((emit_skip == 2 || (emit_skip == 1 && r.cout <= 128)) && r.has_skip && r.mode == 0 && r.conv1.w16 && r.skip.w16 && conv6_supported(Ho, Wo) && conv5_supported(B, r.cout, Ho, Wo) &&
            Cin % 16 == 0 && Cin <= kConv5EmitMaxC && (Ho * Wo) % 256 == 0 && eplane < ((size_t)1 << 32) && !(fuse_small && gn_act_small_supported(Cin, in.H, in.W, 0))) {
            const bool x1 = e->precision == 2;
            float4* prm1 = nullptr;
            TapeRes tr{};
            DPIR_TRY(resolve());
            DPIR_TRY(gn(r.gn1, in, r.name + "#gn1", -1, true, &prm1, &tr.st1));
            tr.prm1 = prm1;
            char* s16 = nullptr;
            DPIR_TRY(ws.getT("act#s16", 2 * eplane, &s16));
            float* sk = nullptr;
            DPIR_TRY(ws.getT(r.name + "#skip", on, &sk));
            Conv5Args a5;
            a5.src = CatSrc{in.a, in.ca, in.b, in.cb}; a5.prm = nullptr; a5.w16 = r.skip.w16; a5.w16_scale = r.skip.w16_scale;
            a5.bias = r.skip.bias; a5.out = sk; a5.res = nullptr; a5.B = B; a5.Cout = r.cout; a5.H = Ho; a5.W = Wo;
            a5.range_ctr = e->range_ctr; a5.x1 = x1;
            a5.emit_prm = prm1; a5.emit_hi = s16; a5.emit_lo = x1 ? nullptr : s16 + eplane;
            fused.erase(sk);
            {
                ProfScope ps(&e->prof, PC_CONV1);
                DPIR_TRY(launch_conv5(s, a5));
            }
            float* o = nullptr;
            DPIR_TRY(ws.getT(r.name + "#out", on, &o));
            if (h1_fusable(r, Ho, Wo)) {
                Conv6Emit em; char* s16b = nullptr; size_t plane2 = 0;
                DPIR_TRY(make_emit(r, Ho, Wo, &em, &s16b, &plane2));
                DPIR_TRY(conv6_on_planes(r.conv1, s16, eplane, nullptr, 0, nullptr, Ho, Wo, &em));
                DPIR_TRY(conv6_on_planes(r.conv2, s16b, plane2, sk, 0, o, Ho, Wo));
            } else {
                DPIR_TRY(conv6_on_planes(r.conv1, s16, eplane, nullptr, 0, h1, Ho, Wo));
                tap(r.name + "#h1", h1, on);
                DPIR_TRY(gn_conv(r.gn2, r.name + "#gn2", r.film_off, r.conv2, h1a, 0, sk, 0, o, Ho, Wo, &tr.prm2, &tr.st2));
            }
            tap(r.name, o, on);
            if (grad) {
                tr.idx = (int)(&r - e->net.res.data());
                tr.in = CatSrc{in.a, in.ca, in.b, in.cb}; tr.inH = in.H; tr.inW = in.W; tr.Ho = Ho; tr.Wo = Wo; tr.h1 = h1; tr.sk = sk; tr.out = o;
                e->tape.nodes.push_back(TapeNode{1, (int)e->tape.res.size()});
                e->tape.res.push_back(tr);
            }
            out->a = o; out->ca = r.cout; out->b = nullptr; out->cb = 0; out->H = Ho; out->W = Wo;
            return Status{};
        }
        TapeRes tr{};
        float* sk = nullptr;
        if (r.has_skip) DPIR_TRY(ws.getT(r.name + "#skip", on, &sk));
        const bool hop9 = fuse_h1 && !grad && r.gn2.c == r.cout && conv9_route(r.conv1, Ho, Wo, true) && conv9_route(r.conv2, Ho, Wo, false);
        const bool fuse = hop9 || h1_fusable(r, Ho, Wo);
        Conv6Emit em; char* s16b = nullptr; size_t plane2 = 0;
        if (hop9) {
            const int C8 = r.cout / 8;
            plane2 = (size_t)B * C8 * Ho * Wo * 16;
            DPIR_TRY(ws.getT("act#s16b", 2 * plane2, &s16b));
            em.hi = s16b; em.lo = e->precision == 2 ? nullptr : s16b + plane2; em.C8 = C8;
            em.gamma = r.gn2.gamma; em.beta = r.gn2.beta;
            em.film = r.film_off >= 0 ? film : nullptr; em.film_stride = film_stride; em.film_off = r.film_off < 0 ? 0 : r.film_off;
            em.frows = film_rows; em.fstep = fstep; em.range_ctr = e->range_ctr;
        } else if (fuse) DPIR_TRY(make_emit(r, Ho, Wo, &em, &s16b, &plane2));
        DPIR_TRY(gn_conv(r.gn1, r.name + "#gn1", -1, r.conv1, in, r.mode, nullptr, 0, fuse ? nullptr : h1, Ho, Wo, &tr.prm1, &tr.st1, fuse ? &em : nullptr));
        if (!fuse) tap(r.name + "#h1", h1, on);
        if (r.has_skip) {
            DPIR_TRY(conv(r.skip, in, 0, nullptr, nullptr, 0, sk, Ho, Wo));
            res = sk;
            tr.sk = sk;
        } else {
            if (in.b) return invalid("resblock " + r.name + ": identity skip on a concatenated input");
            res = in.a; res_mode = r.mode;
        }
        float* o = nullptr;
        DPIR_TRY(ws.getT(r.name + "#out", on, &o));
        if (fuse) DPIR_TRY(conv6_on_planes(r.conv2, s16b, plane2, res, res_mode, o, Ho, Wo));
        else DPIR_TRY(gn_conv(r.gn2, r.name + "#gn2", r.film_off, r.conv2, h1a, 0, res, res_mode, o, Ho, Wo, &tr.prm2, &tr.st2));
        tap(r.name, o, on);
        if (grad) {
            tr.idx = (int)(&r - e->net.res.data());
            tr.in = CatSrc{in.a, in.ca, in.b, in.cb}; tr.inH = in.H; tr.inW = in.W; tr.Ho = Ho; tr.Wo = Wo; tr.h1 = h1; tr.out = o;
            e->tape.nodes.push_back(TapeNode{1, (int)e->tape.res.size()});
            e->tape.res.push_back(tr);
        }
        out->a = o; out->ca = r.cout; out->b = nullptr; out->cb = 0; out->H = Ho; out->W = Wo;
        return Status{};
    }

    Status attention(const AttnW& aw, const Act& in, Act* out) {
        if (in.b || in.ca != aw.c) return invalid("attention " + aw.name + ": bad input");
        int T = in.H * in.W;
        float4* prm = nullptr;
        float2* gst = nullptr;
        DPIR_TRY(resolve());
        DPIR_TRY(gn(aw.norm, in, aw.name + "#norm", -1, false, &prm, &gst));
        float *qkv = nullptr, *att = nullptr, *o = nullptr;
        DPIR_TRY(ws.getT(aw.name + "#qkv", (size_t)B * 3 * aw.c * T, &qkv));
        DPIR_TRY(ws.getT(aw.name + "#att", (size_t)B * aw.c * T, &att));
        DPIR_TRY(ws.getT(aw.name + "#out", (size_t)B * aw.c * T, &o));
        DPIR_TRY(conv(aw.qkv, in, 0, prm, nullptr, 0, qkv, in.H, in.W));
        {
            ProfScope ps(&e->prof, PC_ATTN);
            DPIR_TRY(launch_attention(s, qkv, att, B, aw.c, T, 64));
        }
        Act aa; aa.a = att; aa.ca = aw.c; aa.H = in.H; aa.W = in.W;
        DPIR_TRY(conv(aw.proj, aa, 0, nullptr, in.a, 0, o, in.H, in.W));
        tap(aw.name + "#qkv", qkv, (size_t)B * 3 * aw.c * T);
        tap(aw.name + "#att", att, (size_t)B * aw.c * T);
        tap(aw.name, o, (size_t)B * aw.c * T);
        if (grad) {
            e->tape.nodes.push_back(TapeNode{2, (int)e->tape.attn.size()});
            e->tape.attn.push_back(TapeAttn{(int)(&aw - e->net.attn.data()), in.a, in.H, in.W, qkv, att, o, prm, gst});
        }
        out->a = o; out->ca = aw.c; out->b = nullptr; out->cb = 0; out->H = in.H; out->W = in.W;
        return Status{};
    }

    Status run_block(const UNet& net, const Block& blk, Act in, Act* out) {
        Act cur = in;
        for (const Layer& l : blk) {
            Act nxt;
            if (l.kind == 1) DPIR_TRY(resblock(net.res[l.idx], cur, &nxt));
            else if (l.kind == 2) DPIR_TRY(attention(net.attn[l.idx], cur, &nxt));
            else return invalid("unexpected layer kind");
            cur = nxt;
        }
        *out = cur;
        return Status{};
    }
};
}

Status unet_film_table(dpir_engine* e, const int* t_dev, int n_steps, float* table) {
    UNet& net = e->net;
    if (!net.loaded) return Status{DPIR_ERR_STATE, "dpir_load_unet has not been called"};
    if (net.desc.num_classes > 0) return invalid("FiLM hoisting needs a class-unconditional model");
    const int mc = net.desc.model_channels, ted = 4 * mc;
    float *tmp = nullptr, *semb = nullptr;
    DPIR_TRY(e->ws.getT("embS#tmp", (size_t)n_steps * (mc + ted), &tmp));
    DPIR_TRY(e->ws.getT("embS#semb", (size_t)n_steps * ted, &semb));
    ProfScope ps(&e->prof, PC_ELEM);
    DPIR_TRY(launch_time_embed(e->stream, t_dev, nullptr, net.freqs, net.te_w0, net.te_b0, net.te_w2, net.te_b2, nullptr, n_steps, mc, tmp, semb));
    DPIR_TRY(launch_rows_gemv(e->stream, net.film_w, net.film_b, semb, n_steps, net.film_rows, ted, table));
    return Status{};
}

Status unet_forward(dpir_engine* e, const float* x, const int* t_dev, const int* y_dev, float* out, int B, int H, int W,
                    const float* film_table, const StepDev* film_step, bool uniform_t) {
    UNet& net = e->net;
    if (!net.loaded) return Status{DPIR_ERR_STATE, "dpir_load_unet has not been called"};
    if ((net.desc.num_classes > 0) != (y_dev != nullptr))
        return invalid("must specify y if and only if the model is class-conditional");
    if (B <= 0 || H <= 0 || W <= 0) return invalid("bad batch / image size");
    Workspace& ws = e->ws;
    hipStream_t s = e->stream;
    ProfScope whole(&e->prof, PC_UNET);
    const int mc = net.desc.model_channels, ted = 4 * mc;
    float *tmp = nullptr, *semb = nullptr, *film = nullptr;
    const bool hoisted = film_table != nullptr && film_step != nullptr;
    static const bool one_row_env = !(getenv("DPIR_UNIFORM_T") && atoi(getenv("DPIR_UNIFORM_T")) == 0);
    const bool one_row = one_row_env && !hoisted && uniform_t && net.desc.num_classes == 0 && y_dev == nullptr;
    if (hoisted && net.desc.num_classes > 0) return invalid("hoisted FiLM table with a class-conditional model");
    if (!hoisted) {
        DPIR_TRY(ws.getT("emb#tmp", (size_t)B * (mc + ted), &tmp));
        DPIR_TRY(ws.getT("emb#semb", (size_t)B * ted, &semb));
        DPIR_TRY(ws.getT("emb#film", (size_t)B * net.film_rows, &film));
        ProfScope ps(&e->prof, PC_ELEM);
        const int Be = one_row ? 1 : B;
        DPIR_TRY(launch_time_embed(s, t_dev, y_dev, net.freqs, net.te_w0, net.te_b0, net.te_w2, net.te_b2, net.label_emb, Be, mc, tmp, semb));
        DPIR_TRY(launch_rows_gemv(s, net.film_w, net.film_b, semb, Be, net.film_rows, ted, film));
    }
    float* partial = nullptr;
    size_t partial_cap = (size_t)16 * 1024 * 1024;
    DPIR_TRY(ws.getT("conv#partial", partial_cap, &partial));
    Fwd f{e, s, ws, B, hoisted ? film_table : film, net.film_rows, (hoisted || one_row) ? 0 : net.film_rows, hoisted ? film_step : nullptr, partial, partial_cap};
    {
        static const bool fuse_env = !(getenv("DPIR_FUSE_SMALL") && atoi(getenv("DPIR_FUSE_SMALL")) == 0);
        static const int emit_env = getenv("DPIR_EMIT_SKIP") ? atoi(getenv("DPIR_EMIT_SKIP")) : 1;
        f.grad = e->grad_enabled;
        f.fuse_small = fuse_env;
        f.emit_skip = emit_env;
        static const bool fuse_h1_env = !(getenv("DPIR_FUSE_H1") && atoi(getenv("DPIR_FUSE_H1")) == 0);
        f.fuse_h1 = fuse_h1_env && !e->fuse_h1_off && !f.grad && e->precision != 0;
        if (f.fuse_h1) {
            f.fuse_cap = (size_t)B * 4096;
            DPIR_TRY(ws.getT("fuse#arena", f.fuse_cap, &f.fuse_arena));
            DPIR_HIP(hipMemsetAsync(f.fuse_arena, 0, f.fuse_cap * sizeof(long long), s));
        }
        ++e->fwd_serial;
        if (f.grad) { e->tape.clear(); e->tape.serial = e->fwd_serial; e->tape.B = B; e->tape.H = H; e->tape.W = W; }
    }
    if (e->collect_taps) e->taps.clear();

    std::vector<Act> hs;
    Act h;
    {
        float* o = nullptr;
        size_t on = (size_t)B * net.conv_in.cout * H * W;
        DPIR_TRY(ws.getT("input_blocks.0.0#out", on, &o));
        Act xin; xin.a = x; xin.ca = 3; xin.H = H; xin.W = W;
        DPIR_TRY(f.conv(net.conv_in, xin, 0, nullptr, nullptr, 0, o, H, W));
        f.tap("input_blocks.0.0", o, on);
        h.a = o; h.ca = net.conv_in.cout; h.H = H; h.W = W;
        hs.push_back(h);
        if (f.grad) e->tape.conv_in_out = o;
    }
    for (size_t i = 1; i < net.in_blocks.size(); ++i) {
        Act o;
        DPIR_TRY(f.run_block(net, net.in_blocks[i], h, &o));
        h = o;
        hs.push_back(h);
    }
    {
        Act o;
        DPIR_TRY(f.run_block(net, net.mid, h, &o));
        h = o;
    }
    for (size_t i = 0; i < net.out_blocks.size(); ++i) {
        Act skip = hs.back(); hs.pop_back();
        if (skip.H != h.H || skip.W != h.W) return invalid("skip connection size mismatch (image size not divisible by the UNet stride)");
        Act cat; cat.a = h.a; cat.ca = h.ca; cat.b = skip.a; cat.cb = skip.ca; cat.H = h.H; cat.W = h.W;
        Act o;
        DPIR_TRY(f.run_block(net, net.out_blocks[i], cat, &o));
        h = o;
    }
    float4* fprm = nullptr; float2* fst = nullptr;
    DPIR_TRY(f.gn_conv(net.out_gn, "out#gn", -1, net.out_conv, h, 0, nullptr, 0, out, H, W, &fprm, &fst));
    DPIR_TRY(f.resolve());
    if (f.grad) { e->tape.final_h = h.a; e->tape.final_prm = fprm; e->tape.final_st = fst; e->tape.valid = true; }
    f.tap("out", out, (size_t)B * net.desc.out_channels * H * W);
    return Status{};
}

double unet_flops(const UNet& net, int H, int W, int cls) {
    if (!net.loaded) return 0.0;
    const double mc = net.desc.model_channels, ted = 4 * mc;
    double f3 = 0, f1 = 0, fa = 0, fl = 2 * (mc * ted + ted * ted);
    double h = H, w = W;
    auto res = [&](const ResW& r) {
        if (r.mode == 1) { h *= 2; w *= 2; } else if (r.mode == 2) { h /= 2; w /= 2; }
        f3 += 2.0 * 9 * r.cin * r.cout * h * w + 2.0 * 9 * r.cout * r.cout * h * w;
        fl += 2.0 * ted * 2 * r.cout;
        if (r.has_skip) f1 += 2.0 * r.cin * r.cout * h * w;
    };
    auto att = [&](const AttnW& a) {
        double T = h * w, c = a.c;
        f1 += 2 * c * 3 * c * T + 2 * c * c * T;
        fa += 2 * 2 * T * T * c;
    };
    auto blk = [&](const Block& b) {
        for (const Layer& l : b) {
            if (l.kind == 0) f3 += 2.0 * 9 * 3 * net.conv_in.cout * h * w;
            else if (l.kind == 1) res(net.res[l.idx]);
            else att(net.attn[l.idx]);
        }
    };
    for (auto& b : net.in_blocks) blk(b);
    blk(net.mid);
    for (auto& b : net.out_blocks) blk(b);
    f3 += 2.0 * 9 * net.out_conv.cin * net.out_conv.cout * H * W;
    if (cls == PC_CONV3) return f3;
    if (cls == PC_CONV1) return f1;
    if (cls == PC_ATTN) return fa;
    if (cls == PC_ELEM) return fl;
    return f3 + f1 + fa + fl;
}

}
```

### include/diffpir_debug.h

```cpp
#ifndef DIFFPIR_DEBUG_H
#define DIFFPIR_DEBUG_H
#include "diffpir_engine.h"
#ifdef __cplusplus
extern "C" {
#endif
int dpir_debug_conv_bench(dpir_engine* e, int B, int Cin, int Cout, int H, int W, int ks, int mode, int with_prm,
                          int dbg, int iters, double* ms_out);
int dpir_debug_victim(dpir_engine* e, int lds_bytes, int threads, int blocks, long long spin_ticks, int iters, unsigned long long* bad_out);
int dpir_debug_victim_alu(dpir_engine* e, int mode, int blocks, int iters_in_kernel, int launches, unsigned long long* bad_out);
int dpir_debug_victim_fft_pk(dpir_engine* e, int blocks, int iters_in_kernel, int launches, unsigned long long* bad_out);
int dpir_debug_victim_fft_nopk(dpir_engine* e, int blocks, int iters_in_kernel, int launches, unsigned long long* bad_out);
int dpir_debug_conv7_check(dpir_engine* e, int B, int Cin, int Cout, int H, int W, int res_mode, int x1, int split, int scaled, int iters,
                           double* ms6_out, double* ms7_out, unsigned long long* mismatches_out, float* maxdiff_out, int* ksplit_out);
int dpir_debug_conv7_emit_supported(dpir_engine* e, int B, int Cout, int H, int W, int* capacity_out);
int dpir_debug_conv5_layer(dpir_engine* e, int B, int ca, int cb, int Cout, int H, int W, int tile, const float* xa, const float* xb,
                           const float* w, const float* bias, const float* prm, const float* res, float* out, int* path_out);
typedef struct dpir_debug_conv3_desc {
    int32_t B, ca, cb, Cout, H, W, mode, res_mode, scaled, prologue, route, split, defer, Cout2;
    const float *xa, *xb, *w, *bias, *res, *prm, *gamma, *beta, *film, *gamma2, *beta2, *w2, *bias2;
    float* out; double* stat_out; float* out2;
    int32_t stat_kind_out, path_out, ksplit_out, reserved;
} dpir_debug_conv3_desc;
int dpir_debug_conv3_layer(dpir_engine* e, dpir_debug_conv3_desc* d);
typedef struct dpir_debug_conv9_desc {
    int32_t B, Cin, Cout, H, W, res_mode, hop, Cout2;
    const float *x, *w, *bias, *res, *prm, *gamma2, *beta2, *film2, *w2, *bias2;
    float* out; double* stat_out; float* out2;
    int32_t ran_out, iters;
    double ms_out;
} dpir_debug_conv9_desc;
int dpir_debug_conv9_layer(dpir_engine* e, dpir_debug_conv9_desc* d);
#ifdef __cplusplus
}
#endif
#endif
```

Baseline: 8.832 images/s.

## Fuse nearest upsample into first conv of upsampling resblocks via phase-decomposed weights

```diff
diff --git a/diffpir_amd/_lib.py b/diffpir_amd/_lib.py
--- a/diffpir_amd/_lib.py
+++ b/diffpir_amd/_lib.py
@@ -69,6 +69,12 @@
 
 class Conv9Desc(C.Structure):
     _fields_ = ([(n, C.c_int32) for n in ("B", "Cin", "Cout", "H", "W", "res_mode", "hop", "Cout2")] +
+                [(n, C.c_void_p) for n in ("x", "w", "bias", "res", "prm", "gamma2", "beta2", "film2", "w2", "bias2", "out", "stat_out", "out2")] +
+                [(n, C.c_int32) for n in ("ran_out", "iters")] + [("ms_out", C.c_double)])
+
+
+class ConvUpDesc(C.Structure):
+    _fields_ = ([(n, C.c_int32) for n in ("B", "Cin", "Cout", "Hs", "Ws", "hop", "force_hop", "Cout2", "route", "reserved")] +
                 [(n, C.c_void_p) for n in ("x", "w", "bias", "res", "prm", "gamma2", "beta2", "film2", "w2", "bias2", "out", "stat_out", "out2")] +
                 [(n, C.c_int32) for n in ("ran_out", "iters")] + [("ms_out", C.c_double)])
 
@@ -180,6 +186,10 @@
     d.dpir_debug_conv3_layer.restype = C.c_int
     d.dpir_debug_conv9_layer.argtypes = [C.c_void_p, C.POINTER(Conv9Desc)]
     d.dpir_debug_conv9_layer.restype = C.c_int
+    d.dpir_debug_conv_up_layer.argtypes = [C.c_void_p, C.POINTER(ConvUpDesc)]
+    d.dpir_debug_conv_up_layer.restype = C.c_int
+    d.dpir_debug_conv_up_counts.argtypes = [C.POINTER(C.c_longlong), C.POINTER(C.c_longlong)]
+    d.dpir_debug_conv_up_counts.restype = None
     for n in ("dpir_debug_conv_bench", "dpir_debug_victim", "dpir_debug_victim_alu", "dpir_debug_victim_fft_pk", "dpir_debug_victim_fft_nopk",
               "dpir_debug_conv7_check"):
         getattr(d, n).restype = C.c_int
diff --git a/diffpir_amd/csrc/conv_up.h b/diffpir_amd/csrc/conv_up.h
--- /dev/null
+++ b/diffpir_amd/csrc/conv_up.h
@@ -0,0 +1,27 @@
+#pragma once
+#include "common.h"
+#include "conv6_params.h"
+#include <vector>
+namespace dpir {
+
+struct ConvUpArgs {
+    const void* xhi = nullptr; const void* xlo = nullptr;
+    const void* wup = nullptr; float wup_scale = 1.f;
+    const float* bias = nullptr; float* out = nullptr;
+    const float* res = nullptr;
+    int B = 0, Cin = 0, Cout = 0, Hs = 0, Ws = 0;
+    float2* stat = nullptr;
+    bool x1 = false;
+    const Conv6Emit* emit = nullptr;
+    int min_wg_hop = 0;
+};
+
+long long conv_up_workgroups(int B, int Cout, int Hs, int Ws);
+const char* conv_up_supported(int B, int Cin, int Cout, int Hs, int Ws, bool emit, int min_wg_hop = 0);
+int conv_up_stat_slots(int Hs, int Ws);
+int conv_up_emit_capacity();
+float pack_weights_conv_up(const float* w_oihw, int cout, int cin, std::vector<uint16_t>& out);
+Status launch_conv_up(hipStream_t s, const ConvUpArgs& a);
+void conv_up_launch_counts(long long* plain, long long* hop);
+
+}
diff --git a/diffpir_amd/csrc/conv_up.hip b/diffpir_amd/csrc/conv_up.hip
--- /dev/null
+++ b/diffpir_amd/csrc/conv_up.hip
@@ -0,0 +1,564 @@
+#include "common.h"
+#include <atomic>
+#include "elem.h"
+#include "lds_dma.h"
+#include "conv6_params.h"
+#include "conv_up.h"
+#include <math.h>
+#include <type_traits>
+
+namespace dpir {
+
+typedef float floatx16 __attribute__((ext_vector_type(16)));
+typedef _Float16 half8 __attribute__((ext_vector_type(8)));
+
+template <int I, int N, class F>
+__device__ __forceinline__ void static_for_u(F&& f) {
+    if constexpr (I < N) {
+        f(std::integral_constant<int, I>{});
+        static_for_u<I + 1, N>(f);
+    }
+}
+
+template <int CTRL>
+__device__ __forceinline__ float dpp_row_shr_u(float v) {
+    return __builtin_bit_cast(float, __builtin_amdgcn_update_dpp(0, __builtin_bit_cast(int, v), CTRL, 0xf, 0xf, true));
+}
+
+__device__ __forceinline__ float silu_u(float v) {
+    float e = __builtin_amdgcn_exp2f(v * -1.4426950408889634f);
+    return v * __builtin_amdgcn_rcpf(1.0f + e);
+}
+
+template <bool X1, bool EMIT>
+__global__ __launch_bounds__(256, 2) void conv_up_kernel(Conv6K p) {
+#if defined(__HIP_DEVICE_COMPILE__)
+    constexpr int TW = 32, TH = 8, LW = TW + 2, LH = TH + 2;
+    constexpr int PATCH = LH * LW;
+    constexpr int NPIECE = (2 * PATCH + 63) / 64;
+    constexpr int NXT = (NPIECE + 3) / 4;
+    constexpr int NPL = X1 ? 1 : 2;
+    constexpr int NACT = NPL * NXT;
+    static_assert(NACT <= 6, "two activation pieces per unit in units 0 .. 2: older than the weights requested in units 4 and 5");
+    constexpr int XB = NPIECE * 1024;
+    constexpr int UNITS = 6;
+    extern __shared__ __attribute__((aligned(16))) char smem_u[];
+
+    const int tid = threadIdx.x;
+    const int lane = tid & 63;
+    const int wave = __builtin_amdgcn_readfirstlane(tid >> 6);
+    const int cw = wave & 1, pw = wave >> 1;
+    const int l31 = lane & 31;
+    const int half = lane >> 5;
+
+    int bid = blockIdx.x;
+    if (!EMIT && (gridDim.x & 7) == 0) bid = (bid & 7) * (gridDim.x >> 3) + (bid >> 3);
+    const int tiles_per_img = p.tiles_x * p.tiles_y;
+    int cb, par, ptile;
+    if (EMIT) {
+        const int per_img = 2 * tiles_per_img * p.n_co_blocks;
+        const int r = bid % per_img;
+        cb = r / (2 * tiles_per_img);
+        const int r2 = r - cb * (2 * tiles_per_img);
+        par = r2 & 1;
+        ptile = (bid / per_img) * tiles_per_img + (r2 >> 1);
+    } else {
+        const int nv = 2 * p.n_co_blocks;
+        const int v = bid % nv;
+        par = v & 1;
+        cb = v >> 1;
+        ptile = bid / nv;
+    }
+    const int n0 = ptile / tiles_per_img;
+    const int trem = ptile - n0 * tiles_per_img;
+    const int co_wave = cb * 64 + cw * 32;
+    const bool wave_live = co_wave < p.Cout;
+    const int ty0 = (trem / p.tiles_x) * TH;
+    const int tx0 = (trem % p.tiles_x) * TW;
+    const int HW = p.H * p.W;
+    const int Wo = 2 * p.W, HWo = 4 * HW;
+    const int n_chunks = p.n_chunks_total;
+
+    unsigned x_off[NXT];
+#pragma unroll
+    for (int u = 0; u < NXT; ++u) {
+        int piece = wave + u * 4;
+        if (piece > NPIECE - 1) piece = NPIECE - 1;
+        const int f = piece * 64 + lane;
+        const int kg = f / PATCH;
+        const int e = f - kg * PATCH;
+        const int hy = e / LW, hx = e - hy * LW;
+        const int gy = ty0 + hy - 1, gx = tx0 + hx - 1;
+        const bool ok = kg < 2 && gy >= 0 && gy < p.H && gx >= 0 && gx < p.W;
+        x_off[u] = ok ? ((unsigned)((n0 * p.C8 + kg) * HW + gy * p.W + gx) << 4) : kOutOfRange;
+    }
+    const size_t xplane_bytes = (size_t)p.B * p.C8 * HW * 16;
+    auto dma_x = [&](int chunk, int buf, int q) __attribute__((always_inline)) {
+        const int u = X1 ? q : q >> 1, plane = X1 ? 0 : q & 1;
+        int piece = wave + u * 4;
+        if (piece > NPIECE - 1) piece = NPIECE - 1;
+        const size_t coff = (size_t)chunk * 2 * HW * 16;
+        const __amdgpu_buffer_rsrc_t rx = rsrc_uniform((plane ? p.xlo : p.xhi) + coff, (unsigned)(xplane_bytes - coff));
+        BLDS6(rx, smem_u + buf * 2 * XB + plane * XB + piece * 1024, x_off[u], 0);
+    };
+
+    const int lane_b = l31 + half * PATCH + (4 * pw + par) * LW;
+    const half8* xbase = reinterpret_cast<const half8*>(smem_u) + lane_b;
+
+    const unsigned lane16 = (unsigned)lane * 16u;
+    half8 a_h[4], a_l[4];
+    auto load_a = [&](int chunk, int rec) __attribute__((always_inline)) {
+        const char* base = p.w16 + ((((size_t)chunk * p.n_co_blocks + cb) * 2 + par) * 2 + cw) * (8 * 2048);
+        const __amdgpu_buffer_rsrc_t rw = rsrc_uniform(base, 8 * 2048);
+        const unsigned so = (unsigned)(rec * 2048);
+        a_h[rec & 3] = __builtin_bit_cast(half8, __builtin_amdgcn_raw_buffer_load_b128(rw, lane16, so, 0));
+        if (!X1) a_l[rec & 3] = __builtin_bit_cast(half8, __builtin_amdgcn_raw_buffer_load_b128(rw, lane16, so + 1024u, 0));
+    };
+
+    floatx16 acc[2][4];
+#pragma unroll
+    for (int i = 0; i < 2; ++i)
+#pragma unroll
+        for (int j = 0; j < 4; ++j)
+#pragma unroll
+            for (int r = 0; r < 16; ++r) acc[i][j][r] = 0.f;
+
+    half8 b_h[2][2], b_l[2][2];
+    auto read_b = [&](int buf, int unit, int grp, int set) __attribute__((always_inline)) {
+        const half8* xh = xbase + buf * (2 * XB / 16);
+        const half8* xl = xh + XB / 16;
+        const int uoff = (unit / 3) * LW + (unit % 3);
+#pragma unroll
+        for (int j = 0; j < 2; ++j) {
+            const int o = (grp * 2 + j) * LW + uoff;
+            b_h[set][j] = xh[o];
+            if (!X1) b_l[set][j] = xl[o];
+        }
+    };
+    auto mfma_rec = [&](int b, int grp, int set, int slot) __attribute__((always_inline)) {
+        if (!X1) {
+#pragma unroll
+            for (int j = 0; j < 2; ++j) acc[b][grp * 2 + j] = __builtin_amdgcn_mfma_f32_32x32x16_f16(a_l[slot], b_h[set][j], acc[b][grp * 2 + j], 0, 0, 0);
+#pragma unroll
+            for (int j = 0; j < 2; ++j) acc[b][grp * 2 + j] = __builtin_amdgcn_mfma_f32_32x32x16_f16(a_h[slot], b_l[set][j], acc[b][grp * 2 + j], 0, 0, 0);
+        }
+#pragma unroll
+        for (int j = 0; j < 2; ++j) acc[b][grp * 2 + j] = __builtin_amdgcn_mfma_f32_32x32x16_f16(a_h[slot], b_h[set][j], acc[b][grp * 2 + j], 0, 0, 0);
+    };
+    auto mfma_group = [&](int unit, int grp, int set) __attribute__((always_inline)) {
+        const int pp = unit / 3, c = unit % 3;
+        if (c == 0) mfma_rec(0, grp, set, (pp * 4 + 0) & 3);
+        else if (c == 1) { mfma_rec(0, grp, set, (pp * 4 + 1) & 3); mfma_rec(1, grp, set, (pp * 4 + 2) & 3); }
+        else mfma_rec(1, grp, set, (pp * 4 + 3) & 3);
+    };
+
+    if (!wave_live) {
+#pragma unroll
+        for (int q = 0; q < NACT; ++q) dma_x(0, 0, q);
+        wait_vmcnt<0>();
+        __syncthreads();
+        int it = 0;
+        for (int chunk = 0; chunk + 1 < n_chunks; ++chunk, ++it) {
+#pragma unroll
+            for (int q = 0; q < NACT; ++q) dma_x(chunk + 1, (it & 1) ^ 1, q);
+            wait_vmcnt<0>();
+            __syncthreads();
+        }
+        __syncthreads();
+        return;
+    }
+
+#pragma unroll
+    for (int q = 0; q < NACT; ++q) dma_x(0, 0, q);
+    load_a(0, 0);
+    load_a(0, 1);
+    load_a(0, 2);
+    wait_vmcnt<0>();
+    __syncthreads();
+    read_b(0, 0, 0, 0);
+
+    auto chunk_body = [&](auto more_c, int chunk, int it) __attribute__((always_inline)) {
+        constexpr bool MORE = decltype(more_c)::value;
+        const int cur = it & 1;
+        static_for_u<0, UNITS>([&](auto unit_c) __attribute__((always_inline)) {
+            constexpr int u = decltype(unit_c)::value;
+            read_b(cur, u, 1, 1);
+            __builtin_amdgcn_sched_barrier(0);
+            if (MORE && u < 3) {
+                if (2 * u < NACT) dma_x(chunk + 1, cur ^ 1, 2 * u);
+                if (2 * u + 1 < NACT) dma_x(chunk + 1, cur ^ 1, 2 * u + 1);
+            }
+            if (u == 0) load_a(chunk, 3);
+            else if (u == 1) load_a(chunk, 4);
+            else if (u == 2) { load_a(chunk, 5); load_a(chunk, 6); }
+            else if (u == 3) load_a(chunk, 7);
+            else if (MORE && u == 4) load_a(chunk + 1, 0);
+            else if (MORE && u == 5) { load_a(chunk + 1, 1); load_a(chunk + 1, 2); }
+            __builtin_amdgcn_sched_barrier(0);
+            mfma_group(u, 0, 0);
+            __builtin_amdgcn_sched_barrier(0);
+            if (u + 1 < UNITS) {
+                read_b(cur, u + 1, 0, 0);
+            } else if (MORE) {
+                wait_vmcnt<3 * NPL>();
+                barrier_lds_only();
+                read_b(cur ^ 1, 0, 0, 0);
+            }
+            __builtin_amdgcn_sched_barrier(0);
+            mfma_group(u, 1, 1);
+            __builtin_amdgcn_sched_barrier(0);
+        });
+    };
+    {
+        int it = 0, chunk = 0;
+        for (; chunk + 1 < n_chunks; ++chunk, ++it) chunk_body(std::true_type{}, chunk, it);
+        chunk_body(std::false_type{}, chunk, it);
+    }
+
+    if constexpr (EMIT) {
+        __syncthreads();
+        float* wl = reinterpret_cast<float*>(smem_u) + wave * 512;
+        const float osc = p.out_scale;
+        if (lane < 32) wl[lane] = p.bias[co_wave + lane];
+        __builtin_amdgcn_wave_barrier();
+#pragma unroll
+        for (int r = 0; r < 16; ++r) {
+            const int ch = (r & 3) + 8 * (r >> 2) + 4 * half;
+            const float b = wl[ch];
+            float s1 = 0.f, s2 = 0.f;
+#pragma unroll
+            for (int i = 0; i < 2; ++i)
+#pragma unroll
+                for (int j = 0; j < 4; ++j) {
+                    const float v = acc[i][j][r] * osc + b;
+                    acc[i][j][r] = v;
+                    s1 += v; s2 += v * v;
+                }
+#pragma unroll
+            for (int o = 16; o > 0; o >>= 1) { s1 += __shfl_xor(s1, o, 64); s2 += __shfl_xor(s2, o, 64); }
+            if (l31 == 0) { wl[64 + ch] = s1; wl[128 + ch] = s2; }
+        }
+        __builtin_amdgcn_wave_barrier();
+        const int cg = p.Cout >> 5;
+        const int gpw = 32 / cg;
+        double* gsum = reinterpret_cast<double*>(reinterpret_cast<float*>(smem_u) + 4 * 512);
+        if (lane < gpw) {
+            double s1 = 0.0, s2 = 0.0;
+            for (int k = 0; k < cg; ++k) { s1 += (double)wl[64 + lane * cg + k]; s2 += (double)wl[128 + lane * cg + k]; }
+            gsum[((cw * 2 + pw) * 8 + lane) * 2] = s1;
+            gsum[((cw * 2 + pw) * 8 + lane) * 2 + 1] = s2;
+        }
+        __syncthreads();
+        const int gpb = 2 * gpw;
+        long long* const accb = p.em.acc + ((size_t)n0 * 32 + (size_t)cb * gpb) * 2;
+        if (wave == 0) {
+            const int gl = lane >> 1, t = lane & 1;
+            long long r = 0;
+            if (gl < gpb) {
+                const int c2 = gl / gpw, g = gl - c2 * gpw;
+                const double v = gsum[((c2 * 2 + 0) * 8 + g) * 2 + t] + gsum[((c2 * 2 + 1) * 8 + g) * 2 + t];
+                r = __hip_atomic_fetch_add(accb + gl * 2 + t, __double2ll_rn(v * (t ? 4096.0 : 1048576.0)), __ATOMIC_RELAXED, __HIP_MEMORY_SCOPE_SYSTEM);
+            }
+            asm volatile("s_waitcnt vmcnt(0)" : : "v"((int)r) : "memory");
+            if (lane == 0) {
+                unsigned* cp = p.em.cnt + (size_t)n0 * p.n_co_blocks + cb;
+                const unsigned old = __hip_atomic_fetch_add(cp, 1u, __ATOMIC_RELAXED, __HIP_MEMORY_SCOPE_SYSTEM);
+                asm volatile("" : : "v"(old));
+                int spins = 0;
+                while (__hip_atomic_load(cp, __ATOMIC_RELAXED, __HIP_MEMORY_SCOPE_SYSTEM) < (unsigned)(2 * tiles_per_img + p.em.expect_extra)) {
+                    switch (p.em.sleep_sel) {
+                        case 0: __builtin_amdgcn_s_sleep(2); break;
+                        case 1: __builtin_amdgcn_s_sleep(8); break;
+                        case 3: __builtin_amdgcn_s_sleep(32); break;
+                        case 4: __builtin_amdgcn_s_sleep(64); break;
+                        case 6: __builtin_amdgcn_s_sleep(127); __builtin_amdgcn_s_sleep(127); break;
+                        case 7: __builtin_amdgcn_s_sleep(127); __builtin_amdgcn_s_sleep(127); __builtin_amdgcn_s_sleep(127); __builtin_amdgcn_s_sleep(127); break;
+                        case 2: __builtin_amdgcn_s_sleep(16); break;
+                        default: __builtin_amdgcn_s_sleep(127); break;
+                    }
+                    if (++spins > p.em.spin_limit) { atomicAdd(p.em.range_ctr, 1ull << 40); break; }
+                }
+            }
+        }
+        __syncthreads();
+        if (lane < 32) {
+            const int c = co_wave + lane;
+            const long long* ap = accb + (size_t)((cw * gpw) + lane / cg) * 2;
+            const double S = (double)__hip_atomic_load(ap, __ATOMIC_RELAXED, __HIP_MEMORY_SCOPE_SYSTEM) * (1.0 / 1048576.0);
+            const double SS = (double)__hip_atomic_load(ap + 1, __ATOMIC_RELAXED, __HIP_MEMORY_SCOPE_SYSTEM) * (1.0 / 4096.0);
+            const double cntd = (double)cg * HWo;
+            const double mean = S / cntd;
+            double var = SS / cntd - mean * mean;
+            if (var < 0) var = 0;
+            const float rstd = (float)(1.0 / sqrt(var + 1e-5));
+            float a = rstd * p.em.gamma[c];
+            float b = p.em.beta[c];
+            if (p.em.film) {
+                const float* f = p.em.film + (p.em.fstep ? (size_t)p.em.fstep->i * p.em.frows : 0) + (size_t)n0 * p.em.film_stride + p.em.film_off;
+                const float sc = 1.0f + f[c];
+                const float sh = f[p.Cout + c];
+                a = a * sc;
+                b = b * sc + sh;
+            }
+            reinterpret_cast<float4*>(wl + 192)[lane] = make_float4((float)mean, a, b, 0.f);
+        }
+        __builtin_amdgcn_wave_barrier();
+        typedef _Float16 half4v __attribute__((ext_vector_type(4)));
+        typedef unsigned int u32x2e __attribute__((ext_vector_type(2)));
+        typedef unsigned int u32x4e __attribute__((ext_vector_type(4)));
+        const float4* tab = reinterpret_cast<const float4*>(wl + 192);
+        bool bad = false;
+        auto norm_split = [&](float x, const float4& m, _Float16& h, _Float16& l) __attribute__((always_inline)) {
+            float v = (x - m.x) * m.y + m.z;
+            v = silu_u(v);
+            bad |= !(fabsf(v) <= 65000.f);
+            v = fminf(fmaxf(v, -65000.f), 65000.f);
+            h = (_Float16)v;
+            l = (_Float16)(v - (float)h);
+        };
+#pragma unroll
+        for (int jb = 0; jb < 4; ++jb) {
+            float4 m[4];
+#pragma unroll
+            for (int q = 0; q < 4; ++q) m[q] = tab[8 * jb + 4 * half + q];
+            const int c8 = (co_wave + 8 * jb) >> 3;
+#pragma unroll
+            for (int j = 0; j < 4; ++j) {
+                half4v h0, l0, h1, l1;
+#pragma unroll
+                for (int q = 0; q < 4; ++q) {
+                    _Float16 th, tl;
+                    norm_split(acc[0][j][jb * 4 + q], m[q], th, tl); h0[q] = th; l0[q] = tl;
+                    norm_split(acc[1][j][jb * 4 + q], m[q], th, tl); h1[q] = th; l1[q] = tl;
+                }
+                const u32x2e e_h = __builtin_bit_cast(u32x2e, h0), o_h = __builtin_bit_cast(u32x2e, h1);
+                const u32x2e e_l = __builtin_bit_cast(u32x2e, l0), o_l = __builtin_bit_cast(u32x2e, l1);
+                u32x4e eh, el;
+                {
+                    const auto s0 = __builtin_amdgcn_permlane32_swap(e_h.x, o_h.x, false, false), s1 = __builtin_amdgcn_permlane32_swap(e_h.y, o_h.y, false, false);
+                    eh.x = s0[0]; eh.y = s1[0]; eh.z = s0[1]; eh.w = s1[1];
+                }
+                const size_t eo = (((size_t)n0 * p.em.C8 + c8) * HWo + (size_t)(2 * (ty0 + 4 * pw + j) + par) * Wo + (2 * (tx0 + l31) + half)) << 4;
+                *reinterpret_cast<u32x4e*>(p.em.hi + eo) = eh;
+                if (!X1) {
+                    const auto s0 = __builtin_amdgcn_permlane32_swap(e_l.x, o_l.x, false, false), s1 = __builtin_amdgcn_permlane32_swap(e_l.y, o_l.y, false, false);
+                    el.x = s0[0]; el.y = s1[0]; el.z = s0[1]; el.w = s1[1];
+                    *reinterpret_cast<u32x4e*>(p.em.lo + eo) = el;
+                }
+            }
+        }
+        {
+            const unsigned long long mk = __ballot(bad);
+            if (mk != 0ull && lane == (int)__builtin_ctzll(mk)) atomicAdd(p.em.range_ctr, (unsigned long long)__builtin_popcountll(mk));
+        }
+        return;
+    }
+
+    __syncthreads();
+    constexpr int TS = 68;
+    float* tr = reinterpret_cast<float*>(smem_u) + wave * (32 * TS);
+    const int q4 = lane & 15, rsub = lane >> 4;
+    const float osc = p.out_scale;
+    const bool do_stat = p.stat != nullptr;
+    const size_t img0 = (size_t)n0 * p.Cout;
+    float* const out_base = p.out + img0 * HWo;
+    const void* const stat_base = do_stat ? (const void*)(p.stat + img0 * p.stat_slots) : (const void*)p.bias;
+    const unsigned stat_bytes = do_stat ? 0xFFFFFFFFu : 0u;
+    typedef unsigned int u32x4 __attribute__((ext_vector_type(4)));
+    typedef unsigned int u32x2 __attribute__((ext_vector_type(2)));
+
+    float bv[8];
+    {
+        const __amdgpu_buffer_rsrc_t r_bias = rsrc_uniform(p.bias, (unsigned)p.Cout * 4u);
+#pragma unroll
+        for (int it = 0; it < 8; ++it) bv[it] = as_f32(__builtin_amdgcn_raw_buffer_load_b32(r_bias, (unsigned)(co_wave + it * 4 + rsub) * 4u, 0, 0));
+    }
+    static_for_u<0, 4>([&](auto j_c) __attribute__((always_inline)) {
+        constexpr int j = decltype(j_c)::value;
+#pragma unroll
+        for (int b = 0; b < 2; ++b)
+#pragma unroll
+            for (int r = 0; r < 16; ++r)
+                tr[((r & 3) + 8 * (r >> 2) + 4 * half) * TS + 2 * l31 + b] = acc[b][j][r] * osc;
+        const unsigned pix = (unsigned)((2 * (ty0 + 4 * pw + j) + par) * Wo + 2 * tx0 + q4 * 4);
+        const int slot = (trem * 2 + par) * 8 + pw * 4 + j;
+        const __amdgpu_buffer_rsrc_t r_out = rsrc_uniform(out_base, 0xFFFFFFFFu);
+        const __amdgpu_buffer_rsrc_t r_stat = rsrc_uniform(stat_base, stat_bytes);
+#pragma unroll
+        for (int it = 0; it < 8; ++it) {
+            const int co_l = it * 4 + rsub;
+            const int co = co_wave + co_l;
+            const bool ok = co < p.Cout;
+            float4 v = *reinterpret_cast<const float4*>(tr + co_l * TS + q4 * 4);
+            v.x += bv[it]; v.y += bv[it]; v.z += bv[it]; v.w += bv[it];
+            if (!ok) v = make_float4(0.f, 0.f, 0.f, 0.f);
+            u32x4 sv;
+            sv.x = as_u32(v.x); sv.y = as_u32(v.y); sv.z = as_u32(v.z); sv.w = as_u32(v.w);
+            __builtin_amdgcn_raw_buffer_store_b128(sv, r_out, ok ? ((unsigned)co * (unsigned)HWo + pix) * 4u : kOutOfRange, 0, 0);
+            if (do_stat) {
+                float s1 = (v.x + v.y) + (v.z + v.w);
+                float s2 = (v.x * v.x + v.y * v.y) + (v.z * v.z + v.w * v.w);
+                s1 += dpp_row_shr_u<0x111>(s1); s2 += dpp_row_shr_u<0x111>(s2);
+                s1 += dpp_row_shr_u<0x112>(s1); s2 += dpp_row_shr_u<0x112>(s2);
+                s1 += dpp_row_shr_u<0x114>(s1); s2 += dpp_row_shr_u<0x114>(s2);
+                s1 += dpp_row_shr_u<0x118>(s1); s2 += dpp_row_shr_u<0x118>(s2);
+                u32x2 st;
+                st.x = as_u32(s1); st.y = as_u32(s2);
+                const bool wr = q4 == 15 && ok;
+                __builtin_amdgcn_raw_buffer_store_b64(st, r_stat, wr ? ((unsigned)co * (unsigned)p.stat_slots + (unsigned)slot) * 8u : kOutOfRange, 0, 0);
+            }
+        }
+    });
+#endif
+}
+
+constexpr size_t kConvUpLds = (size_t)4 * ((2 * 10 * 34 + 63) / 64) * 1024;
+static_assert(kConvUpLds >= 4 * 32 * 68 * 4 && kConvUpLds >= 4 * 512 * 4 + 2 * 2 * 8 * 2 * 8, "epilogue slabs / hop scratch");
+static_assert(2 * kConvUpLds <= 160 * 1024, "two workgroups per CU");
+
+template <bool X1, bool EMIT>
+static Status launch_up(hipStream_t s, const Conv6K& k, int blocks) {
+    auto fn = conv_up_kernel<X1, EMIT>;
+    static LdsAttrOnce attr_set;
+    DPIR_HIP(attr_set.set(reinterpret_cast<const void*>(fn), (int)kConvUpLds));
+    hipLaunchKernelGGL(fn, dim3((unsigned)blocks), dim3(256), kConvUpLds, s, k);
+    return Status{};
+}
+
+int conv_up_emit_capacity() {
+    static std::atomic<int> caps[16];
+    int dev = 0, cus = 0, occ = 0;
+    if (hipGetDevice(&dev) != hipSuccess) return 0;
+    std::atomic<int>* slot = (dev >= 0 && dev < 16) ? &caps[dev] : nullptr;
+    if (slot && slot->load() > 0) return slot->load() - 1;
+    if (hipDeviceGetAttribute(&cus, hipDeviceAttributeMultiprocessorCount, dev) != hipSuccess) return 0;
+    if (hipOccupancyMaxActiveBlocksPerMultiprocessor(&occ, conv_up_kernel<false, true>, 256, kConvUpLds) != hipSuccess || occ < 1) occ = 1;
+    if (occ > 2) occ = 2;
+    if (slot) slot->store(cus * occ + 1);
+    return cus * occ;
+}
+
+long long conv_up_workgroups(int B, int Cout, int Hs, int Ws) {
+    return (long long)B * (Ws / 32) * (Hs / 8) * ((Cout + 63) / 64) * 2;
+}
+
+int conv_up_stat_slots(int Hs, int Ws) { return (Ws / 32) * (Hs / 8) * 16; }
+
+const char* conv_up_supported(int B, int Cin, int Cout, int Hs, int Ws, bool emit, int min_wg_hop) {
+    if (B <= 0 || Cin <= 0 || Cout <= 0 || Hs <= 0 || Ws <= 0) return "conv_up: bad shape";
+    if (Ws & 31) return "conv_up: the source width must be a multiple of 32";
+    if (Hs & 7) return "conv_up: the source height must be a multiple of 8";
+    if (Cin & 15) return "conv_up: the input channels must be a multiple of 16";
+    if (Cout & 31) return "conv_up: the output channels must be a multiple of 32";
+    const size_t HW = (size_t)Hs * Ws;
+    if ((size_t)B * (Cin / 8) * HW * 16 >= ((size_t)1 << 32) || (size_t)Cout * HW * 16 >= ((size_t)1 << 32) ||
+        conv_up_workgroups(B, Cout, Hs, Ws) >= ((long long)1 << 31))
+        return "conv_up: operand planes or one image's output exceed the 4 GiB buffer-descriptor range";
+    if (emit) {
+        if ((Cout & 63) || 32 % (Cout / 32) != 0) return "conv_up: GroupNorm groups of the hop must not straddle a wave's 32 channels (Cout 128, 256, 512 or 1024)";
+        const int wait_set = 2 * (Ws / 32) * (Hs / 8);
+        if (wait_set > conv_up_emit_capacity() / 2) return "conv_up: the hop's wait set exceeds half of the resident workgroups";
+        if (conv_up_workgroups(B, Cout, Hs, Ws) < min_wg_hop) return "conv_up: too few workgroups for the hop";
+        if ((size_t)B * (Cout / 8) * HW * 4 * 16 >= ((size_t)1 << 32)) return "conv_up: the emitted planes exceed the 4 GiB range";
+    }
+    return nullptr;
+}
+
+static std::atomic<long long> g_launches[2];
+void conv_up_launch_counts(long long* plain, long long* hop) {
+    if (plain) *plain = g_launches[0].load();
+    if (hop) *hop = g_launches[1].load();
+}
+
+Status launch_conv_up(hipStream_t s, const ConvUpArgs& a) {
+    if (a.res) return invalid("conv_up: conv1 of an up-sampling ResBlock takes no residual");
+    if (const char* why = conv_up_supported(a.B, a.Cin, a.Cout, a.Hs, a.Ws, a.emit != nullptr, a.min_wg_hop)) return Status{DPIR_ERR_UNSUPPORTED, why};
+    if (!a.xhi || (!a.x1 && !a.xlo) || !a.wup || !a.bias || (!a.emit && !a.out)) return invalid("conv_up: null operand");
+    Conv6K k{};
+    k.xhi = reinterpret_cast<const char*>(a.xhi); k.xlo = reinterpret_cast<const char*>(a.xlo);
+    k.w16 = reinterpret_cast<const char*>(a.wup); k.bias = a.bias; k.out = a.out; k.res = nullptr; k.res_mode = 0;
+    k.B = a.B; k.Cout = a.Cout; k.H = a.Hs; k.W = a.Ws;
+    k.n_chunks_total = a.Cin / 16;
+    k.C8 = 2 * k.n_chunks_total;
+    k.tiles_x = a.Ws / 32; k.tiles_y = a.Hs / 8;
+    k.n_co_blocks = (a.Cout + 63) / 64;
+    k.ksplit = 1; k.chunks_per_split = k.n_chunks_total; k.partial = nullptr; k.zeros = nullptr;
+    k.out_scale = 1.0f / a.wup_scale; k.out_scale_dev = nullptr;
+    k.stat = a.emit ? nullptr : a.stat; k.stat_slots = conv_up_stat_slots(a.Hs, a.Ws);
+    const int blocks = (int)conv_up_workgroups(a.B, a.Cout, a.Hs, a.Ws);
+    if (a.emit) {
+        if (!a.emit->hi || (!a.x1 && !a.emit->lo) || !a.emit->acc || !a.emit->cnt || !a.emit->range_ctr || !a.emit->gamma || !a.emit->beta)
+            return invalid("conv_up: the hop needs planes, accumulators, counters, the range guard and the GroupNorm affine");
+        k.em = *a.emit;
+        DPIR_TRY((a.x1 ? launch_up<true, true>(s, k, blocks) : launch_up<false, true>(s, k, blocks)));
+    } else {
+        DPIR_TRY((a.x1 ? launch_up<true, false>(s, k, blocks) : launch_up<false, false>(s, k, blocks)));
+    }
+    DPIR_HIP(hipGetLastError());
+    ++g_launches[a.emit ? 1 : 0];
+    return Status{};
+}
+
+static _Float16 f16_nearest(double v) {
+    _Float16 best = (_Float16)(float)v;
+    uint16_t bits;
+    __builtin_memcpy(&bits, &best, 2);
+    for (int d = -1; d <= 1; d += 2) {
+        const uint16_t nb = (uint16_t)(bits + d);
+        if ((nb & 0x7C00) == 0x7C00 || ((nb ^ bits) & 0x8000)) continue;
+        _Float16 c;
+        __builtin_memcpy(&c, &nb, 2);
+        const double eb = fabs(v - (double)best), ec = fabs(v - (double)c);
+        if (ec < eb || (ec == eb && (nb & 1) == 0)) best = c;
+    }
+    return best;
+}
+
+float pack_weights_conv_up(const float* w, int cout, int cin, std::vector<uint16_t>& out) {
+    const int chunks = (cin + 15) / 16, cblocks = (cout + 63) / 64;
+    auto taps_of = [](int par, int t, int& k0, int& k1) {
+        if (par == 0) { k0 = t == 0 ? 0 : 1; k1 = t == 0 ? 0 : 2; }
+        else { k0 = t == 0 ? 0 : 2; k1 = t == 0 ? 1 : 2; }
+    };
+    auto combined = [&](int co, int ci, int a, int b, int pp, int q) -> double {
+        int y0, y1, x0, x1;
+        taps_of(a, pp, y0, y1);
+        taps_of(b, q, x0, x1);
+        double s = 0.0;
+        for (int ky = y0; ky <= y1; ++ky)
+            for (int kx = x0; kx <= x1; ++kx) s += (double)w[((size_t)co * cin + ci) * 9 + ky * 3 + kx];
+        return s;
+    };
+    double mxd = 0.0;
+    for (int co = 0; co < cout; ++co)
+        for (int ci = 0; ci < cin; ++ci)
+            for (int v = 0; v < 16; ++v) mxd = fmax(mxd, fabs(combined(co, ci, v >> 3, (v >> 2) & 1, (v >> 1) & 1, v & 1)));
+    const float mx = (float)mxd;
+    float scale = 1.0f;
+    if (mx > 0.f) scale = exp2f(floorf(log2f(1024.0f / mx)));
+    while (mx * scale >= 1024.0f) scale *= 0.5f;
+    out.assign((size_t)chunks * cblocks * 2 * 2 * 8 * 1024, 0);
+    for (int ch = 0; ch < chunks; ++ch)
+        for (int cbk = 0; cbk < cblocks; ++cbk)
+            for (int a = 0; a < 2; ++a)
+                for (int wv = 0; wv < 2; ++wv)
+                    for (int rec = 0; rec < 8; ++rec) {
+                        const int pp = rec >> 2, b = (rec >> 1) & 1, q = rec & 1;
+                        uint16_t* hi = out.data() + ((((((size_t)ch * cblocks + cbk) * 2 + a) * 2 + wv) * 8) + rec) * 1024;
+                        uint16_t* lo = hi + 512;
+                        for (int kh = 0; kh < 2; ++kh)
+                            for (int col = 0; col < 32; ++col)
+                                for (int j = 0; j < 8; ++j) {
+                                    const int co = cbk * 64 + wv * 32 + col, ci = ch * 16 + kh * 8 + j;
+                                    const double v = (co < cout && ci < cin) ? combined(co, ci, a, b, pp, q) * (double)scale : 0.0;
+                                    const _Float16 h = f16_nearest(v);
+                                    const _Float16 l = f16_nearest(v - (double)h);
+                                    const size_t o = ((size_t)kh * 32 + col) * 8 + j;
+                                    __builtin_memcpy(&hi[o], &h, 2);
+                                    __builtin_memcpy(&lo[o], &l, 2);
+                                }
+                    }
+    return scale;
+}
+
+}
diff --git a/diffpir_amd/csrc/dbg_conv.hip b/diffpir_amd/csrc/dbg_conv.hip
--- a/diffpir_amd/csrc/dbg_conv.hip
+++ b/diffpir_amd/csrc/dbg_conv.hip
@@ -1,6 +1,7 @@
 #include "engine.h"
 #include "conv6_params.h"
 #include "conv9.h"
+#include "conv_up.h"
 #include "../../include/diffpir_debug.h"
 #include <string.h>
 #include <vector>
@@ -595,6 +596,141 @@
     return DPIR_OK;
 }
 
+int dpir_debug_conv_up_layer(dpir_engine* e, dpir_debug_conv_up_desc* d) {
+    if (!e || !d) return DPIR_ERR_INVALID;
+    d->ran_out = 0; d->ms_out = 0.0;
+    const int B = d->B, Cin = d->Cin, Cout = d->Cout, Hs = d->Hs, Ws = d->Ws;
+    if (!d->x || !d->w || !d->bias || B <= 0 || Cin <= 0 || Cout <= 0 || Hs <= 0 || Ws <= 0 || (!d->hop && !d->out) || d->route < 0 || d->route > 1 ||
+        (d->hop && (!d->gamma2 || !d->beta2 || !d->w2 || !d->bias2 || !d->out2 || d->Cout2 <= 0)))
+        return fail(e, invalid("conv_up layer: bad descriptor"));
+    if (e->grad_enabled) return fail(e, Status{DPIR_ERR_UNSUPPORTED, "conv_up layer: a gradient-mode engine keeps launch_conv6's route"});
+    if (e->precision == 0) return fail(e, Status{DPIR_ERR_UNSUPPORTED, "conv_up layer: the f32 precision keeps the fp32 kernel"});
+    if (d->res) return fail(e, invalid("conv_up: conv1 of an up-sampling ResBlock takes no residual"));
+    const int min_wg = d->force_hop ? 0 : 384;
+    if (d->route == 0) {
+        if (const char* why = conv_up_supported(B, Cin, Cout, Hs, Ws, d->hop != 0, min_wg)) return fail(e, Status{DPIR_ERR_UNSUPPORTED, why});
+    } else if (Cin % 16 || !conv6_supported(2 * Hs, 2 * Ws) || (d->hop && !conv7_emit_supported(B, Cout, 2 * Hs, 2 * Ws))) {
+        return fail(e, Status{DPIR_ERR_UNSUPPORTED, "conv_up layer: launch_conv6's route refuses this shape"});
+    }
+    (void)hipSetDevice(e->device);
+    const bool x1 = e->precision == 2;
+    const int H = 2 * Hs, W = 2 * Ws;
+    const size_t HWs = (size_t)Hs * Ws, HW = 4 * HWs, nx = (size_t)B * Cin * HWs, no = (size_t)B * Cout * HW;
+    const int C8 = 2 * ((Cin + 15) / 16);
+    const size_t plane_s = (size_t)B * C8 * HWs * 16, plane = 4 * plane_s;
+    const int slots = conv_up_stat_slots(Hs, Ws);
+    const size_t nst = (size_t)B * Cout * slots;
+    float *dx = nullptr, *dbias = nullptr, *dout = nullptr; float4* dprm = nullptr; float2* st = nullptr; char* s16 = nullptr;
+    API_TRY(e, e->ws.getT("cu#x", nx, &dx));
+    API_TRY(e, e->ws.getT("cu#b", (size_t)round_up(Cout, 64), &dbias));
+    API_TRY(e, e->ws.getT("cu#o", no, &dout));
+    API_TRY(e, e->ws.getT("cu#prm", (size_t)B * Cin, &dprm));
+    API_TRY(e, e->ws.getT("cu#st", nst, &st));
+    API_TRY(e, e->ws.getT("cu#s16", 2 * plane, &s16));
+    API_HIP(e, hipMemcpy(dx, d->x, nx * 4, hipMemcpyHostToDevice));
+    API_HIP(e, hipMemset(dbias, 0, (size_t)round_up(Cout, 64) * 4));
+    API_HIP(e, hipMemcpy(dbias, d->bias, (size_t)Cout * 4, hipMemcpyHostToDevice));
+    if (d->prm) API_HIP(e, hipMemcpy(dprm, d->prm, (size_t)B * Cin * 16, hipMemcpyHostToDevice));
+    API_HIP(e, hipMemsetAsync(dout, 0xFF, no * 4, e->stream));
+    API_HIP(e, hipMemsetAsync(st, 0xFF, nst * 8, e->stream));
+    API_HIP(e, hipMemsetAsync(s16, 0xFF, 2 * plane, e->stream));
+    std::vector<uint16_t> wv;
+    const float w_scale = d->route == 0 ? pack_weights_conv_up(d->w, Cout, Cin, wv) : pack_weights_conv6(d->w, Cout, Cin, wv);
+    void* wp = nullptr;
+    API_TRY(e, e->ws.get("cu#w", wv.size() * 2, &wp));
+    API_HIP(e, hipMemcpy(wp, wv.data(), wv.size() * 2, hipMemcpyHostToDevice));
+    const CatSrc src{dx, Cin, nullptr, 0};
+    const float4* prm = d->prm ? dprm : nullptr;
+    const int Co2 = d->hop ? d->Cout2 : 0, C8b = 2 * ((Cout + 15) / 16);
+    const size_t plane2 = (size_t)B * C8b * HW * 16, no2 = (size_t)B * Co2 * HW;
+    char* s16b = nullptr; float *dg = nullptr, *db = nullptr, *df = nullptr, *dbias2 = nullptr, *dout2 = nullptr; long long* arena = nullptr; void* wp2 = nullptr;
+    const size_t arena_words = (size_t)B * 64 + ((size_t)B * ((Cout + 63) / 64) + 1) / 2;
+    Conv6Emit em;
+    float w2_scale = 1.f;
+    if (d->hop) {
+        API_TRY(e, e->ws.getT("cu#s16b", 2 * plane2, &s16b));
+        API_TRY(e, e->ws.getT("cu#gamma2", (size_t)Cout, &dg));
+        API_TRY(e, e->ws.getT("cu#beta2", (size_t)Cout, &db));
+        API_TRY(e, e->ws.getT("cu#film2", (size_t)B * 2 * Cout, &df));
+        API_TRY(e, e->ws.getT("cu#b2", (size_t)round_up(Co2, 64), &dbias2));
+        API_TRY(e, e->ws.getT("cu#o2", no2, &dout2));
+        API_TRY(e, e->ws.getT("cu#arena", arena_words, &arena));
+        API_HIP(e, hipMemsetAsync(s16b, 0xFF, 2 * plane2, e->stream));
+        API_HIP(e, hipMemcpy(dg, d->gamma2, (size_t)Cout * 4, hipMemcpyHostToDevice));
+        API_HIP(e, hipMemcpy(db, d->beta2, (size_t)Cout * 4, hipMemcpyHostToDevice));
+        if (d->film2) API_HIP(e, hipMemcpy(df, d->film2, (size_t)B * 2 * Cout * 4, hipMemcpyHostToDevice));
+        API_HIP(e, hipMemset(dbias2, 0, (size_t)round_up(Co2, 64) * 4));
+        API_HIP(e, hipMemcpy(dbias2, d->bias2, (size_t)Co2 * 4, hipMemcpyHostToDevice));
+        API_HIP(e, hipMemsetAsync(dout2, 0xFF, no2 * 4, e->stream));
+        std::vector<uint16_t> w16b;
+        w2_scale = pack_weights_conv6(d->w2, Co2, Cout, w16b);
+        API_TRY(e, e->ws.get("cu#w16b", w16b.size() * 2, &wp2));
+        API_HIP(e, hipMemcpy(wp2, w16b.data(), w16b.size() * 2, hipMemcpyHostToDevice));
+        em.hi = s16b; em.lo = x1 ? nullptr : s16b + plane2; em.C8 = C8b; em.gamma = dg; em.beta = db;
+        em.film = d->film2 ? df : nullptr; em.film_stride = 2 * Cout; em.film_off = 0; em.frows = 2 * Cout; em.fstep = nullptr;
+        em.acc = arena; em.cnt = reinterpret_cast<unsigned*>(arena + (size_t)B * 64); em.range_ctr = e->range_ctr;
+    }
+    int kernel1 = 0;
+    auto once = [&]() -> Status {
+        if (d->hop) DPIR_HIP(hipMemsetAsync(arena, 0, arena_words * 8, e->stream));
+        if (d->route == 0) {
+            DPIR_TRY(launch_act_split(e->stream, src, prm, 0, B, Hs, Ws, s16, x1 ? nullptr : s16 + plane_s, e->range_ctr));
+            ConvUpArgs a;
+            a.xhi = s16; a.xlo = s16 + plane_s; a.wup = wp; a.wup_scale = w_scale; a.bias = dbias; a.out = d->hop ? nullptr : dout;
+            a.B = B; a.Cin = Cin; a.Cout = Cout; a.Hs = Hs; a.Ws = Ws; a.stat = d->hop ? nullptr : st; a.x1 = x1;
+            a.emit = d->hop ? &em : nullptr; a.min_wg_hop = min_wg;
+            DPIR_TRY(launch_conv_up(e->stream, a));
+        } else {
+            DPIR_TRY(launch_act_split(e->stream, src, prm, 1, B, H, W, s16, x1 ? nullptr : s16 + plane, e->range_ctr));
+            Conv6Args a6;
+            a6.x1 = x1; a6.xhi = s16; a6.xlo = s16 + plane; a6.w16 = wp; a6.w16_scale = w_scale; a6.bias = dbias; a6.out = d->hop ? nullptr : dout;
+            a6.B = B; a6.Cin = Cin; a6.Cout = Cout; a6.H = H; a6.W = W; a6.stat = d->hop ? nullptr : st;
+            a6.emit = d->hop ? &em : nullptr;
+            int kind = 0;
+            DPIR_TRY(launch_conv6(e->stream, a6, &kind, nullptr, &kernel1));
+            if (!d->hop && kind != 1) return invalid("conv_up layer: launch_conv6 produced no epilogue statistics here");
+        }
+        if (d->hop) {
+            Conv6Args c6;
+            c6.x1 = x1; c6.xhi = s16b; c6.xlo = s16b + plane2; c6.w16 = wp2; c6.w16_scale = w2_scale;
+            c6.bias = dbias2; c6.out = dout2; c6.B = B; c6.Cin = Cout; c6.Cout = Co2; c6.H = H; c6.W = W;
+            DPIR_TRY(launch_conv6(e->stream, c6));
+        }
+        return Status{};
+    };
+    API_TRY(e, once());
+    if (d->iters > 0) {
+        hipEvent_t e0, e1;
+        API_HIP(e, hipEventCreate(&e0)); API_HIP(e, hipEventCreate(&e1));
+        API_HIP(e, hipEventRecord(e0, e->stream));
+        for (int i = 0; i < d->iters; ++i) API_TRY(e, once());
+        API_HIP(e, hipEventRecord(e1, e->stream));
+        API_HIP(e, hipEventSynchronize(e1));
+        float ms = 0; API_HIP(e, hipEventElapsedTime(&ms, e0, e1));
+        (void)hipEventDestroy(e0); (void)hipEventDestroy(e1);
+        d->ms_out = ms / d->iters;
+    }
+    API_HIP(e, hipStreamSynchronize(e->stream));
+    d->ran_out = d->route == 0 ? (d->hop ? 2 : 1) : 7;
+    if (d->hop) {
+        API_HIP(e, hipMemcpy(d->out2, dout2, no2 * 4, hipMemcpyDeviceToHost));
+        return DPIR_OK;
+    }
+    API_HIP(e, hipMemcpy(d->out, dout, no * 4, hipMemcpyDeviceToHost));
+    if (d->stat_out) {
+        std::vector<float2> hs(nst);
+        API_HIP(e, hipMemcpy(hs.data(), st, nst * 8, hipMemcpyDeviceToHost));
+        for (size_t pl = 0; pl < (size_t)B * Cout; ++pl) {
+            double s1 = 0.0, s2 = 0.0;
+            for (int k = 0; k < slots; ++k) { s1 += (double)hs[pl * slots + k].x; s2 += (double)hs[pl * slots + k].y; }
+            d->stat_out[2 * pl] = s1; d->stat_out[2 * pl + 1] = s2;
+        }
+    }
+    return DPIR_OK;
+}
+
+void dpir_debug_conv_up_counts(long long* plain, long long* hop) { conv_up_launch_counts(plain, hop); }
+
 int dpir_debug_conv7_emit_supported(dpir_engine* e, int B, int Cout, int H, int W, int* capacity_out) {
     if (!e) return 0;
     (void)hipSetDevice(e->device);
diff --git a/diffpir_amd/csrc/engine.h b/diffpir_amd/csrc/engine.h
--- a/diffpir_amd/csrc/engine.h
+++ b/diffpir_amd/csrc/engine.h
@@ -30,7 +30,8 @@
                void* w16 = nullptr; float w16_scale = 1.f;
                float* wT = nullptr; int coutpT = 0;
                void* w8 = nullptr; float w8_scale = 1.f;
-               void* w16T = nullptr; float w16T_scale = 1.f; };
+               void* w16T = nullptr; float w16T_scale = 1.f;
+               void* wup = nullptr; float wup_scale = 1.f; };
 struct GnW { float* gamma = nullptr; float* beta = nullptr; int c = 0; };
 struct ResW {
     std::string name;
diff --git a/diffpir_amd/csrc/unet.hip b/diffpir_amd/csrc/unet.hip
--- a/diffpir_amd/csrc/unet.hip
+++ b/diffpir_amd/csrc/unet.hip
@@ -1,6 +1,7 @@
 #include "engine.h"
 #include "conv6_params.h"
 #include "conv9.h"
+#include "conv_up.h"
 #include <unordered_map>
 #include <cstdint>
 #include <math.h>
@@ -55,7 +56,7 @@
     return Status{};
 }
 
-Status load_conv(dpir_engine* e, const WeightMap& wm, const std::string& p, int cin, int cout, int ks, bool one_d, ConvW* out) {
+Status load_conv(dpir_engine* e, const WeightMap& wm, const std::string& p, int cin, int cout, int ks, bool one_d, ConvW* out, bool up_pack = false) {
     const float *w = nullptr, *b = nullptr;
     std::vector<int64_t> shape = one_d ? std::vector<int64_t>{cout, cin, 1} : std::vector<int64_t>{cout, cin, ks, ks};
     DPIR_TRY(wm.find(p + ".weight", shape, &w));
@@ -112,6 +113,15 @@
             DPIR_HIP(hipMemcpy(p8, w8.data(), w8.size() * 2, hipMemcpyHostToDevice));
             out->w8 = p8;
         }
+        if (up_pack && ks == 3 && !one_d && cin % 16 == 0 && cout % 32 == 0) {
+            std::vector<uint16_t> wu;
+            out->wup_scale = pack_weights_conv_up(w, cout, cin, wu);
+            void* pu = nullptr;
+            if (hipMalloc(&pu, wu.size() * 2) != hipSuccess) return Status{DPIR_ERR_NOMEM, "hipMalloc for the phase weights failed"};
+            e->net.allocs.push_back(pu);
+            DPIR_HIP(hipMemcpy(pu, wu.data(), wu.size() * 2, hipMemcpyHostToDevice));
+            out->wup = pu;
+        }
     }
     return Status{};
 }
@@ -157,7 +167,7 @@
     auto add_res = [&](const std::string& p, int cin, int cout, int mode, Block& blk) -> Status {
         ResW r; r.name = p; r.cin = cin; r.cout = cout; r.mode = mode;
         DPIR_TRY(load_gn(e, wm, p + ".in_layers.0", cin, &r.gn1));
-        DPIR_TRY(load_conv(e, wm, p + ".in_layers.2", cin, cout, 3, false, &r.conv1));
+        DPIR_TRY(load_conv(e, wm, p + ".in_layers.2", cin, cout, 3, false, &r.conv1, mode == 1));
         DPIR_TRY(load_gn(e, wm, p + ".out_layers.0", cout, &r.gn2));
         DPIR_TRY(load_conv(e, wm, p + ".out_layers.3", cout, cout, 3, false, &r.conv2));
         r.has_skip = cin != cout;
@@ -490,7 +500,8 @@
                conv7_emit_supported(B, r.cout, Ho, Wo) && fuse_arena && fuse_off + (size_t)B * 64 + (size_t)B * (r.cout / 128) <= fuse_cap &&
                (size_t)B * (2 * ((r.cout + 15) / 16)) * Ho * Wo * 16 < ((size_t)1 << 32);
     }
-    Status make_emit(const ResW& r, int Ho, int Wo, Conv6Emit* em, char** s16b, size_t* plane2) {
+    Status make_emit(const ResW& r, int Ho, int Wo, Conv6Emit* em, char** s16b, size_t* plane2, int cnt_per_img = 0) {
+        if (cnt_per_img <= 0) cnt_per_img = r.cout / 128;
         const bool x1 = e->precision == 2;
         const int C8 = 2 * ((r.cout + 15) / 16);
         *plane2 = (size_t)B * C8 * Ho * Wo * 16;
@@ -502,7 +513,7 @@
         em->acc = fuse_arena + fuse_off;
         fuse_off += (size_t)B * 64;
         em->cnt = reinterpret_cast<unsigned*>(fuse_arena + fuse_off);
-        fuse_off += ((size_t)B * (r.cout / 128) + 1) / 2;
+        fuse_off += ((size_t)B * cnt_per_img + 1) / 2;
         em->range_ctr = e->range_ctr;
         static const int spin_env = getenv("DPIR_FUSE_SPIN_LIMIT") ? atoi(getenv("DPIR_FUSE_SPIN_LIMIT")) : 0;
         static const int extra_env = getenv("DPIR_FUSE_EXPECT_EXTRA") ? atoi(getenv("DPIR_FUSE_EXPECT_EXTRA")) : 0;
@@ -510,6 +521,73 @@
         em->sleep_sel = sleep_env;
         if (spin_env > 0) em->spin_limit = spin_env;
         em->expect_extra = extra_env;
+        return Status{};
+    }
+
+    bool conv_up_route(const ResW& r, const Act& in) const {
+        static const bool on = !(getenv("DPIR_CONV_UP") && atoi(getenv("DPIR_CONV_UP")) == 0);
+        return on && r.mode == 1 && !grad && e->precision != 0 && r.conv1.wup && !in.b && in.C() == r.gn1.c &&
+               !conv_up_supported(B, in.C(), r.cout, in.H, in.W, false) && conv_up_workgroups(B, r.cout, in.H, in.W) >= 256;
+    }
+    Status resblock_up(const ResW& r, const Act& in, Act* out, int Ho, int Wo, float* h1, size_t on) {
+        const bool x1 = e->precision == 2;
+        const int C = in.C(), C8 = 2 * (C / 16);
+        const size_t plane = (size_t)B * C8 * in.H * in.W * 16;
+        char* s16 = nullptr;
+        DPIR_TRY(ws.getT("act#s16", 2 * plane, &s16));
+        if (fuse_small && gn_act_small_supported(C, in.H, in.W, 0)) {
+            if (pending.partial && !is_pending(in.a)) DPIR_TRY(resolve());
+            GnActArgs ga;
+            ga.src = CatSrc{in.a, in.ca, nullptr, 0};
+            ga.pend = pending;
+            ga.gamma = r.gn1.gamma; ga.beta = r.gn1.beta;
+            ga.film = nullptr; ga.film_stride = film_stride; ga.film_off = 0; ga.fstep = fstep; ga.frows = film_rows;
+            ga.silu = true; ga.mode = 0; ga.B = B; ga.Hs = in.H; ga.Ws = in.W;
+            ga.hi = s16; ga.lo = x1 ? nullptr : s16 + plane; ga.range_ctr = e->range_ctr;
+            {
+                ProfScope ps(&e->prof, PC_ELEM);
+                DPIR_TRY(launch_gn_act_small(s, ga));
+            }
+            if (pending.partial) { fused.erase(pending.out); pending = PendingConv{}; }
+        } else {
+            DPIR_TRY(resolve());
+            float4* prm = nullptr;
+            DPIR_TRY(gn(r.gn1, in, r.name + "#gn1", -1, true, &prm));
+            ProfScope ps(&e->prof, PC_ELEM);
+            DPIR_TRY(launch_act_split(s, CatSrc{in.a, in.ca, nullptr, 0}, prm, 0, B, in.H, in.W, s16, x1 ? nullptr : s16 + plane, e->range_ctr));
+        }
+        ConvUpArgs a;
+        a.xhi = s16; a.xlo = s16 + plane; a.wup = r.conv1.wup; a.wup_scale = r.conv1.wup_scale; a.bias = r.conv1.bias;
+        a.B = B; a.Cin = C; a.Cout = r.cout; a.Hs = in.H; a.Ws = in.W; a.x1 = x1;
+        float* o = nullptr;
+        DPIR_TRY(ws.getT(r.name + "#out", on, &o));
+        const bool hop = fuse_h1 && r.gn2.c == r.cout && r.conv2.w16 && r.conv2.ks == 3 && conv6_supported(Ho, Wo) && fuse_arena &&
+                         !conv_up_supported(B, C, r.cout, in.H, in.W, true, 384) && fuse_off + (size_t)B * 64 + (size_t)B * (r.cout / 64) <= fuse_cap;
+        if (hop) {
+            Conv6Emit em; char* s16b = nullptr; size_t plane2 = 0;
+            DPIR_TRY(make_emit(r, Ho, Wo, &em, &s16b, &plane2, r.cout / 64));
+            a.emit = &em; a.min_wg_hop = 384;
+            {
+                ProfScope ps(&e->prof, PC_CONV3);
+                DPIR_TRY(launch_conv_up(s, a));
+            }
+            DPIR_TRY(conv6_on_planes(r.conv2, s16b, plane2, in.a, 1, o, Ho, Wo));
+        } else {
+            const int slots = conv_up_stat_slots(in.H, in.W);
+            float2* st = nullptr;
+            DPIR_TRY(ws.getT("st#" + std::to_string(reinterpret_cast<uintptr_t>(h1)), (size_t)B * r.cout * slots, &st));
+            a.out = h1; a.stat = st;
+            {
+                ProfScope ps(&e->prof, PC_CONV3);
+                DPIR_TRY(launch_conv_up(s, a));
+            }
+            fused[h1] = FusedStat{st, slots, nullptr};
+            tap(r.name + "#h1", h1, on);
+            Act h1a; h1a.a = h1; h1a.ca = r.cout; h1a.H = Ho; h1a.W = Wo;
+            DPIR_TRY(gn_conv(r.gn2, r.name + "#gn2", r.film_off, r.conv2, h1a, 0, in.a, 1, o, Ho, Wo));
+        }
+        tap(r.name, o, on);
+        out->a = o; out->ca = r.cout; out->b = nullptr; out->cb = 0; out->H = Ho; out->W = Wo;
         return Status{};
     }
 
@@ -521,6 +599,7 @@
         size_t on = (size_t)B * r.cout * Ho * Wo;
         float* h1 = nullptr;
         DPIR_TRY(ws.getT(r.name + "#h1", on, &h1));
+        if (conv_up_route(r, in)) return resblock_up(r, in, out, Ho, Wo, h1, on);
         Act h1a; h1a.a = h1; h1a.ca = r.cout; h1a.H = Ho; h1a.W = Wo;
         const float* res = nullptr; int res_mode = 0;
         const int Cin = in.C();
diff --git a/include/diffpir_debug.h b/include/diffpir_debug.h
--- a/include/diffpir_debug.h
+++ b/include/diffpir_debug.h
@@ -30,6 +30,15 @@
     double ms_out;
 } dpir_debug_conv9_desc;
 int dpir_debug_conv9_layer(dpir_engine* e, dpir_debug_conv9_desc* d);
+typedef struct dpir_debug_conv_up_desc {
+    int32_t B, Cin, Cout, Hs, Ws, hop, force_hop, Cout2, route, reserved;
+    const float *x, *w, *bias, *res, *prm, *gamma2, *beta2, *film2, *w2, *bias2;
+    float* out; double* stat_out; float* out2;
+    int32_t ran_out, iters;
+    double ms_out;
+} dpir_debug_conv_up_desc;
+int dpir_debug_conv_up_layer(dpir_engine* e, dpir_debug_conv_up_desc* d);
+void dpir_debug_conv_up_counts(long long* plain, long long* hop);
 #ifdef __cplusplus
 }
 #endif
```

New measurement: 9.264 images/s, median of 6. 4.9% higher.
